# troylee/nnet-asr

Hardware: AMD Instinct MI355X
Metric: training frames/sec (whole node), 440→2048×4→senone MLP, 1/2/4/8 MI355X (higher is better)
Workload: dtype f32; 1 GPU; TNet SGD step, 440x2048x2048x2048x2048x4000 sigmoid MLP + softmax xent; bunch_per_gpu=1024, global_bunch=1024, frames_resident_per_gpu=65536, parallelism=dp1

## Files before the change

### include/tnet_kernels.h

```cpp
#ifndef TNET_KERNELS_H_
#define TNET_KERNELS_H_

#ifdef __cplusplus
extern "C" {
#endif

typedef struct TnetMatrixDim_ {
  int rows;
  int cols;
  int stride;
} TnetMatrixDim;

#define TNET_STATS_SLOTS 512
#define TNET_STATS_WORDS (2 * TNET_STATS_SLOTS)

enum {
  TNET_OK = 0,
  TNET_ERR_ARG = -1,
  TNET_ERR_LAUNCH = -2,
  TNET_ERR_RUNTIME = -3,
  TNET_ERR_UNSUPPORTED = -4
};

const char* tnet_status_str(int status);
// ... 10 lines not shown
int tnetF_add_scaled_row(float alpha, const float* row, float beta, float* dst, TnetMatrixDim d, void* stream);
int tnetF_mul_elem(float* mat, const float* A, int strideA, TnetMatrixDim d, void* stream);
int tnetF_log_elem(float* mat, TnetMatrixDim d, void* stream);

long tnet_col_sum_workspace(TnetMatrixDim d);
int tnetF_add_col_sum(float alpha, const float* mat, float beta, float* vec, TnetMatrixDim d, void* workspace,
                      void* stream);

int tnetF_sigmoid(float* y, const float* x, TnetMatrixDim d, void* stream);
int tnetF_diff_sigmoid(float* eout, const float* e, const float* y, TnetMatrixDim d, void* stream);
int tnetF_softmax(float* y, const float* x, TnetMatrixDim d, void* stream);
int tnetF_check_class(const float* out, const float* des, int* match, TnetMatrixDim d, void* stream);

int tnetF_expand(float* y, const float* x, const int* off, TnetMatrixDim dout, TnetMatrixDim din, void* stream);
int tnetF_rearrange(float* y, const float* x, const int* copy_from, TnetMatrixDim dout, TnetMatrixDim din,
                    void* stream);
int tnet_block_linearity(float* y, TnetMatrixDim dy, const float* x, TnetMatrixDim dx, const float* t,
                         TnetMatrixDim dt, void* stream);
int tnetF_randomize(float* y, const float* x, const int* copy_from, TnetMatrixDim dout, TnetMatrixDim din,
                    void* stream);
int tnet_gather_i32(int* out, const int* in, const int* copy_from, int n, void* stream);
int tnet_gather_bunch(float* y, const float* x, int* labels_out, const int* labels_in, const int* copy_from,
                      TnetMatrixDim dout, TnetMatrixDim din, void* stream);

int tnet_sgemm(char transa, char transb, int m, int n, int k, float alpha, const float* A, int lda,
               const float* B, int ldb, float beta, float* C, int ldc, void* stream);
int tnet_gemm_config(const char* name);
int tnet_gemm_reserve(int cus);

int tnet_affine_fwd(const float* X, TnetMatrixDim dX, const float* W, TnetMatrixDim dW, const float* b,
                    float* Y, TnetMatrixDim dY, int act, void* stream);
int tnet_affine_fwd_sample(const float* X, TnetMatrixDim dX, const float* W, TnetMatrixDim dW, const float* b,
                           float* Y, TnetMatrixDim dY, float* states, int ld_states, unsigned* z1, unsigned* z2,
                           unsigned* z3, unsigned* z4, void* stream);
int tnet_affine_fwd_t(const float* X, TnetMatrixDim dX, const float* W, TnetMatrixDim dW, const float* b,
                      float* Y, TnetMatrixDim dY, int act, void* stream);
int tnet_affine_bwd(const float* E, TnetMatrixDim dE, const float* W, TnetMatrixDim dW, const float* Ybelow,
                    int strideYbelow, float* Eo, TnetMatrixDim dEo, int dsig, void* stream);
int tnet_affine_update(const float* X, TnetMatrixDim dX, const float* E, TnetMatrixDim dE, float* W,
                       TnetMatrixDim dW, float* corrW, int strideCorr, float scale, float mmt, float l2,
                       void* stream);
int tnet_colsum_slabs(int rows);
int tnet_affine_bwd_colsum(const float* E, TnetMatrixDim dE, const float* W, TnetMatrixDim dW,
                           const float* Ybelow, int strideYbelow, float* Eo, TnetMatrixDim dEo, float* colpart,
                           int ldcolpart, void* stream);
int tnet_colsum_slab_sums(const float* E, TnetMatrixDim dE, float* colpart, int ldcolpart, void* stream);
#define TNET_AFFINE_SOFTMAX_MAX_N 256
int tnet_affine_softmax_xent(const float* X, TnetMatrixDim dX, const float* W, TnetMatrixDim dW, const float* b,
                             const int* labels, float* Z, int strideZ, float* Y, int strideY, float* E, int strideE,
                             double* stats, float* colpart, int ldcolpart, void* stream);
int tnet_affine_update_bias(const float* X, TnetMatrixDim dX, const float* E, TnetMatrixDim dE, float* W,
                            TnetMatrixDim dW, float* corrW, int strideCorr, float scale, float mmt, float l2,
                            const float* colpart, int ldcolpart, float* b, float* corr_b, void* stream);
int tnet_affine_update_bwd_pair(const float* X, TnetMatrixDim dX, const float* E, TnetMatrixDim dE, float* W,
                                TnetMatrixDim dW, float* corrW, int strideCorr, float scale, float mmt, float l2,
                                const float* colpart, int ldcolpart, float* b, float* corr_b, const float* E2,
                                TnetMatrixDim dE2, const float* W2, TnetMatrixDim dW2, const float* Ybelow,
                                int strideYbelow, float* Eo, TnetMatrixDim dEo, float* colpart2, int ldcolpart2,
                                void* stream);
int tnet_affine_update_bias_pair(const float* X, TnetMatrixDim dX, const float* E, TnetMatrixDim dE, float* W,
                                 TnetMatrixDim dW, float* corrW, int strideCorr, float scale, float mmt, float l2,
                                 const float* colpart, int ldcolpart, float* b, float* corr_b, const float* X2,
                                 TnetMatrixDim dX2, const float* E2, TnetMatrixDim dE2, float* W2, TnetMatrixDim dW2,
                                 float* corrW2, int strideCorr2, float scale2, float mmt2, float l22,
                                 const float* colpart2, int ldcolpart2, float* b2, float* corr_b2, void* stream);
int tnet_affine_bwd_colsum_slabs(const float* E, TnetMatrixDim dE, const float* W, TnetMatrixDim dW,
                                 const float* Ybelow, int strideYbelow, float* Eo, TnetMatrixDim dEo, float* colpart,
                                 int ldcolpart, float* colpartE, int ldcolpartE, void* stream);
int tnet_affine_bwd_colsum_t(const float* E, TnetMatrixDim dE, const float* Wt, TnetMatrixDim dWt, const float* Ybelow,
                             int strideYbelow, float* Eo, TnetMatrixDim dEo, float* colpart, int ldcolpart,
                             void* stream);
int tnet_affine_bwd_colsum_slabs_t(const float* E, TnetMatrixDim dE, const float* Wt, TnetMatrixDim dWt,
                                   const float* Ybelow, int strideYbelow, float* Eo, TnetMatrixDim dEo, float* colpart,
                                   int ldcolpart, float* colpartE, int ldcolpartE, void* stream);
int tnet_affine_update_bwd_pair_t(const float* X, TnetMatrixDim dX, const float* E, TnetMatrixDim dE, float* W,
                                  TnetMatrixDim dW, float* corrW, int strideCorr, float scale, float mmt, float l2,
                                  const float* colpart, int ldcolpart, float* b, float* corr_b, const float* E2,
                                  TnetMatrixDim dE2, const float* W2t, TnetMatrixDim dW2t, const float* Ybelow,
                                  int strideYbelow, float* Eo, TnetMatrixDim dEo, float* colpart2, int ldcolpart2,
                                  void* stream);
int tnet_weight_shadow(const float* W, TnetMatrixDim dW, float* Wt, int ldwt);
int tnet_weight_shadow_kept(const float* W);
int tnet_transpose(const float* A, TnetMatrixDim dA, float* T, int ldt, void* stream);
int tnet_affine_update_bias_gather(const float* X, TnetMatrixDim dX, const float* E, TnetMatrixDim dE, float* W,
                                   TnetMatrixDim dW, float* corrW, int strideCorr, float scale, float mmt, float l2,
                                   const float* colpart, int ldcolpart, float* b, float* corr_b, const float* X2,
                                   TnetMatrixDim dX2, const float* E2, TnetMatrixDim dE2, float* W2,
                                   TnetMatrixDim dW2, float* corrW2, int strideCorr2, float scale2, float mmt2,
                                   float l22, const float* colpart2, int ldcolpart2, float* b2, float* corr_b2,
                                   float* y, const float* x, int* labels_out, const int* labels_in,
                                   const int* copy_from, TnetMatrixDim dy, TnetMatrixDim dx, void* stream);
int tnet_affine_grad(const float* X, TnetMatrixDim dX, const float* E, TnetMatrixDim dE, float* G,
                     TnetMatrixDim dG, void* stream);
int tnet_affine_grad_bias(const float* X, TnetMatrixDim dX, const float* E, TnetMatrixDim dE, float* G,
                          TnetMatrixDim dG, const float* colpart, int ldcolpart, float* gradB, void* stream);
int tnet_affine_grad_bwd_pair(const float* X, TnetMatrixDim dX, const float* E, TnetMatrixDim dE, float* G,
                              TnetMatrixDim dG, const float* colpart, int ldcolpart, float* gradB, const float* E2,
                              TnetMatrixDim dE2, const float* W2, TnetMatrixDim dW2, const float* Ybelow,
                              int strideYbelow, float* Eo, TnetMatrixDim dEo, float* colpart2, int ldcolpart2,
                              void* stream);
int tnet_affine_grad_bias_gather(const float* X, TnetMatrixDim dX, const float* E, TnetMatrixDim dE, float* G,
                                 TnetMatrixDim dG, const float* colpart, int ldcolpart, float* gradB, const float* X2,
                                 TnetMatrixDim dX2, const float* E2, TnetMatrixDim dE2, float* G2, TnetMatrixDim dG2,
                                 const float* colpart2, int ldcolpart2, float* gradB2, float* y, const float* x,
                                 int* labels_out, const int* labels_in, const int* copy_from, TnetMatrixDim dy,
                                 TnetMatrixDim dx, void* stream);
int tnet_sgd_update(float* p, const float* g, float* corr, long n, float scale, float mmt, float l2,
                    void* stream);
typedef struct TnetSgdSeg_ {
  float* p;
  const float* g;
  float* corr;
  long n;
  float l2;
} TnetSgdSeg;
int tnet_sgd_update_multi(const TnetSgdSeg* segs, int nseg, float scale, float mmt, void* stream);
int tnet_bias_update(const float* E, TnetMatrixDim dE, float* b, float* corr_b, float* grad_out, float scale,
                     float mmt, void* workspace, void* stream);
int tnet_rbm_update(const float* V, TnetMatrixDim dV, const float* H, TnetMatrixDim dH, float* W,
                    TnetMatrixDim dW, float* corrW, int strideCorr, float scale, float mmt, float l2,
                    void* stream);
int tnet_rbm_bias_update(const float* M, TnetMatrixDim d, int neg_from, float* b, float* corr_b, float scale,
                         float mmt, void* workspace, void* stream);
int tnet_rbm_update_stats(const float* V, TnetMatrixDim dV, const float* H, TnetMatrixDim dH, float* W,
                          TnetMatrixDim dW, float* corrW, int strideCorr, float scale, float mmt, float l2, int B,
                          float* vb, float* cvb, float* hb, float* chb, double* mse_stats, void* stream);
int tnet_rbm_update_stats_gather(const float* V, TnetMatrixDim dV, const float* H, TnetMatrixDim dH, float* W,
                                 TnetMatrixDim dW, float* corrW, int strideCorr, float scale, float mmt, float l2,
                                 int B, float* vb, float* cvb, float* hb, float* chb, double* mse_stats, float* y,
                                 const float* x, int* labels_out, const int* labels_in, const int* copy_from,
                                 TnetMatrixDim dy, TnetMatrixDim dx, void* stream);
int tnet_rbm_stats_update(const float* Vs, TnetMatrixDim dV, const float* Hs, TnetMatrixDim dH, int B, float* vb,
                          float* cvb, float* hb, float* chb, float scale, float mmt, double* mse_stats, void* stream);

int tnet_gemv_rowvec_cat(const float* v0, int K0, const float* v1, int K1, float* vout, const float* W, int ldw,
                         const float* b, float* y, int N, int act, void* workspace, void* stream);
int tnet_gemv_rowvec_softmax_xent(const float* v, int K, const float* W, int ldw, const float* b, float* z, float* y,
                                  float* e, int N, const int* label, double* stats, void* workspace, void* stream);
int tnet_gemv_rowvec_partial(const float* v0, int K0, const float* v1, int K1, float* vout, const float* W, int ldw,
                             int N, float* partial, void* stream);
int tnet_rnn_out_partial(const float* hpart, int hslices, const float* hb, float* h, int H, const float* Wo, int ldwo,
                         int N, float* opart, void* stream);
int tnet_rnn_out_stats(const float* opart, int H, int N, const float* bo, float* z, double* smx, void* stream);
int tnet_rnn_out_full(const float* hpart, int hslices, const float* hb, float* h, int H, const float* Wo, int ldwo,
                      int N, const float* bo, float* z, double* smx, void* stream);
int tnet_gemv_rowvec_partial_update(const float* v0, int K0, const float* v1, int K1, float* vout, float* W, int ldw,
                                    int N, float* partial, const float* hist, int ldh, int head, int R, const float* D,
                                    int ldd, int steps, float* b, float* corr_b, float lr, float mmt, float wc,
                                    void* stream);
int tnet_rnn_out_bwd_update(const float* z, const double* smx, int pairs, int N, const int* label, const float* h,
                            int H, float* Wo, int ldwo, float* corrWo, int ldc, float* bo, float* corr_bo, float scale,
                            float mmt, float l2, float* y, float* e, float* e_out, float* d, double* stats,
                            unsigned long long* argkey, int train, void* stream);
int tnet_argmax_correct(const unsigned long long* keys, const int* labels, int T, int N, double* stats,
                        void* stream);
int tnet_rnn_out_full_ahead(const float* hpart, int hslices, const float* hb, float* h, int H, const float* Wo,
                            int ldwo, int N, const float* bo, float* z, double* smx, const float* dpart, const float* D,
                            int ldd, int steps, float lr, float mmt, float wc, const float* cb, float* bnext,
                            float* cbnext, float* W, int ldw, int rows, const float* hist, int ldh, int head, int R,
                            void* stream);
int tnet_rnn_out_bwd_update_ahead(const float* z, const double* smx, int pairs, int N, const int* label,
                                  const float* h, int H, float* Wo, int ldwo, float* corrWo, int ldc, float* bo,
                                  float* corr_bo, float scale, float mmt, float l2, float* e, float* eo, float* d,
                                  double* stats, unsigned long long* argkey, const float* bnext, const float* cbnext,
                                  float* b, float* cb, const float* x_next, int nIn, const float* W, int ldw,
                                  float* partial, float* dpart, float* vout, const float* hist, int ldh, int head,
// ... 78 lines not shown
```

### include/tnet_train.h

```cpp
#ifndef TNET_TRAIN_H_
#define TNET_TRAIN_H_

#include <stddef.h>

#include "tnet_kernels.h"

#ifdef __cplusplus
extern "C" {
#endif

typedef struct TnetNetwork TnetNetwork;
typedef struct TnetObjective TnetObjective;
typedef struct TnetTrainer TnetTrainer;
typedef struct TnetComm TnetComm;
typedef struct TnetRbmTrainer TnetRbmTrainer;
typedef struct TnetRnnTrainer TnetRnnTrainer;

const char* tnet_last_error(void);

int tnet_device_count(int* n);
int tnet_select_gpu(int gpu_id);
int tnet_synchronize(void);
void* tnet_stream(void);
int tnet_malloc(void** p, size_t bytes);
int tnet_free(void* p);
int tnet_memcpy_h2d(void* dst, const void* src, size_t bytes);
int tnet_memcpy_d2h(void* dst, const void* src, size_t bytes);
int tnet_memcpy_d2d(void* dst, const void* src, size_t bytes);
int tnet_memset(void* dst, int value, size_t bytes);
int tnet_set_profile(int on);
int tnet_profile_report(char* buf, int cap);
int tnet_kernel_timing(int on);
int tnet_kernel_timing_filter(const char* filter);
int tnet_kernel_timing_report(char* buf, int cap);
int tnet_timer_start(void);
int tnet_timer_stop(float* ms);

TnetNetwork* tnet_net_read(const char* path);
TnetNetwork* tnet_net_read_text(const char* text);
int tnet_net_write(TnetNetwork* net, const char* path);
int tnet_net_free(TnetNetwork* net);
int tnet_net_num_components(TnetNetwork* net);
int tnet_net_component(TnetNetwork* net, int i, char* tag, int cap, int* n_in, int* n_out);
int tnet_net_get_params(TnetNetwork* net, int i, float* W, float* b);
int tnet_net_set_params(TnetNetwork* net, int i, const float* W, const float* b);
int tnet_net_set_learn_rate(TnetNetwork* net, float lr, const char* factors);
int tnet_net_set_momentum(TnetNetwork* net, float mmt);
int tnet_net_set_weightcost(TnetNetwork* net, float wc);
int tnet_net_set_grad_div_frm(TnetNetwork* net, int div);
int tnet_net_propagate(TnetNetwork* net, const float* dX, int rows, int ldx, float* dY, int ldy);
int tnet_net_backpropagate(TnetNetwork* net, const float* dE, int rows, int lde);
int tnet_net_train_bunch(TnetNetwork* net, TnetObjective* obj, const float* dX, int rows, int ldx,
                         const int* dLabels, int train);
int tnet_net_keep_output(TnetNetwork* net, int keep);
int tnet_net_output(TnetNetwork* net, int i, float* host, int ld);

TnetObjective* tnet_obj_create(int type);
int tnet_obj_free(TnetObjective* obj);
int tnet_obj_evaluate(TnetObjective* obj, const float* dOut, int rows, int cols, int ldo, const float* dDes,
                      int ldd, float* dErr, int lde);
int tnet_obj_evaluate_labels(TnetObjective* obj, const float* dOut, int rows, int cols, int ldo,
                             const int* dLabels, float* dErr, int lde);
int tnet_obj_stats(TnetObjective* obj, double* error, long* frames, double* correct);
int tnet_obj_report(TnetObjective* obj, char* buf, int cap);
int tnet_obj_reset(TnetObjective* obj);

TnetTrainer* tnet_trainer_create(TnetNetwork* net, TnetObjective* obj, int bunchsize, int cachesize, long seed,
                                 int randomize, int crossval);
int tnet_trainer_free(TnetTrainer* t);
int tnet_trainer_add_utterance(TnetTrainer* t, const float* feats, int rows, int cols, int ld, const int* labels);
int tnet_trainer_finish(TnetTrainer* t);
long tnet_trainer_steps(TnetTrainer* t);
int tnet_trainer_replay(TnetTrainer* t, long nsteps);
long tnet_trainer_prefill(TnetTrainer* t, const float* feats, int rows, int cols, int ld, const int* labels);
int tnet_debug_fail_train_bunch(long n);
int tnet_trainer_set_comm(TnetTrainer* t, TnetComm* comm);
long tnet_trainer_empty_steps(TnetTrainer* t);
int tnet_trainer_trace(TnetTrainer* t, int trace);
int tnet_trainer_set_transform(TnetTrainer* t, TnetNetwork* transform, int start_ext, int end_ext);

typedef struct TnetFeatureReader TnetFeatureReader;
TnetFeatureReader* tnet_reader_create(const char* scp, int swap, int start_ext, int end_ext, int target_kind,
                                      int deriv_order, const int* deriv_win, const char* mlf, const char* label_map,
                                      const char* label_dir, const char* label_ext, int threads, int depth);
TnetFeatureReader* tnet_reader_create_norm(const char* scp, int swap, int start_ext, int end_ext, int target_kind,
                                           int deriv_order, const int* deriv_win, const char* mlf,
                                           const char* label_map, const char* label_dir, const char* label_ext,
                                           const char* cmn_dir, const char* cmn_mask, const char* cvn_dir,
                                           const char* cvn_mask, const char* cvg_file, int threads, int depth);
int tnet_reader_free(TnetFeatureReader* r);
long tnet_reader_size(TnetFeatureReader* r);
int tnet_reader_next(TnetFeatureReader* r, const float** feats, int* rows, int* cols, const int** labels,
                     int* n_labels, int* samp_period, int* kind, char* logical, int logical_cap);
int tnet_reader_rewind(TnetFeatureReader* r);
int tnet_htk_read(const char* record, int swap, int start_ext, int end_ext, float* out, long cap, int* rows, int* cols,
                  int* samp_period, int* kind);
int tnet_mask_match(const char* mask, const char* label, char* captured, int cap);
int tnet_mlf_lookup(const char* const* patterns, int n_patterns, const char* const* labels, int n_labels,
                    int* rec_out);
long tnet_trainer_add_reader(TnetTrainer* t, TnetFeatureReader* r, long max_utts);

int tnet_net_rbm_get(TnetNetwork* net, int i, float* W, float* vis_bias, float* hid_bias, int* types);
int tnet_net_rbm_set(TnetNetwork* net, int i, const float* W, const float* vis_bias, const float* hid_bias,
                     int vis_type, int hid_type);
int tnet_net_rbm_update(TnetNetwork* net, int i, const float* pos_vis, const float* pos_hid, const float* neg_vis,
                        const float* neg_hid, int rows, int ld_vis, int ld_hid);
TnetRbmTrainer* tnet_rbm_trainer_create(TnetNetwork* net, int bunchsize, int cachesize, long seed, int randomize,
                                        float learn_rate, float momentum, float weightcost);
int tnet_rbm_trainer_free(TnetRbmTrainer* t);
int tnet_rbm_trainer_add_utterance(TnetRbmTrainer* t, const float* feats, int rows, int cols, int ld);
int tnet_rbm_trainer_finish(TnetRbmTrainer* t);
long tnet_rbm_trainer_steps(TnetRbmTrainer* t);
int tnet_rbm_trainer_stats(TnetRbmTrainer* t, double* mse, long* frames);
int tnet_rbm_trainer_report(TnetRbmTrainer* t, char* buf, int cap);
long tnet_rbm_trainer_prefill(TnetRbmTrainer* t, const float* feats, int rows, int cols, int ld);
int tnet_rbm_trainer_replay(TnetRbmTrainer* t, long nsteps);

int tnet_net_recurrent_get(TnetNetwork* net, int i, float* W, float* b);
int tnet_net_recurrent_set(TnetNetwork* net, int i, const float* W, const float* b);
TnetRnnTrainer* tnet_rnn_trainer_create(TnetNetwork* net, TnetObjective* obj, int bptt, int crossval);
int tnet_rnn_trainer_free(TnetRnnTrainer* t);
int tnet_rnn_trainer_utterance(TnetRnnTrainer* t, const float* feats, int rows, int cols, int ld, const int* labels);
long tnet_rnn_trainer_frames(TnetRnnTrainer* t);

int tnet_net_shared_get(TnetNetwork* net, int i, float* W, float* b, int* n_inst);
int tnet_net_shared_set(TnetNetwork* net, int i, const float* W, const float* b);

int tnet_net_discrete_blocks(TnetNetwork* net, int i, int* n_blocks, int* n_in, int* n_out);
// ... 32 lines not shown
```

### nnet-asr_amd/csrc/host/capi.cpp

```cpp
#include <cstring>
#include <fstream>
#include <memory>
#include <sstream>
#include <string>

#include "tnet_train.h"
#include "curbm.h"
#include "curecurrent.h"
#include "cudiscrete.h"
#include "cushared.h"
#include "cusparse.h"
#include "htkio.h"
#include "trainer.h"

using namespace TNet;

static thread_local std::string g_last_error;

#define TRY_BEGIN try {
#define TRY_END                              \
  }                                          \
  catch (std::exception & e) {               \
    g_last_error = e.what();                 \
    return TNET_ERR_RUNTIME;                 \
// ... 121 lines not shown
  TRY_END
}

int tnet_kernel_timing(int on) {
  TRY_BEGIN CuDevice::Instantiate().KernelTiming(on == 2 ? 2 : on != 0 ? 1 : 0);
  TRY_END
}
int tnet_kernel_timing_filter(const char* filter) {
  TRY_BEGIN CuDevice::Instantiate().KernelTimingFilter(filter ? filter : "");
  TRY_END
}
int tnet_kernel_timing_report(char* buf, int cap) {
  TRY_BEGIN std::string s = CuDevice::Instantiate().KTCollect();
  if ((int)s.size() >= cap) Error("tnet_kernel_timing_report: buffer too small");
  std::strncpy(buf, s.c_str(), (size_t)cap);
  TRY_END
}

static hipEvent_t g_t0 = nullptr, g_t1 = nullptr;
int tnet_timer_start(void) {
  TRY_BEGIN if (!g_t0) {
    TNET_HIP_CALL(hipEventCreate(&g_t0));
    TNET_HIP_CALL(hipEventCreate(&g_t1));
  }
  TNET_HIP_CALL(hipEventRecord(g_t0, CuDevice::Instantiate().Stream()));
  TRY_END
}
int tnet_timer_stop(float* ms) {
  TRY_BEGIN TNET_HIP_CALL(hipEventRecord(g_t1, CuDevice::Instantiate().Stream()));
  TNET_HIP_CALL(hipEventSynchronize(g_t1));
  TNET_HIP_CALL(hipEventElapsedTime(ms, g_t0, g_t1));
  TRY_END
}

TnetNetwork* tnet_net_read(const char* path) {
  try {
    std::unique_ptr<TnetNetwork> h(new TnetNetwork);
    h->net.ReadNetwork(path);
    return h.release();
  }
  TRY_END_PTR
}
TnetNetwork* tnet_net_read_text(const char* text) {
  try {
    std::unique_ptr<TnetNetwork> h(new TnetNetwork);
    std::istringstream is(text);
    h->net.ReadNetwork(is);
    return h.release();
  }
  TRY_END_PTR
}
int tnet_net_write(TnetNetwork* h, const char* path) {
  TRY_BEGIN h->net.WriteNetwork(path);
  TRY_END
}
int tnet_net_free(TnetNetwork* h) {
  TRY_BEGIN delete h;
  TRY_END
}
int tnet_net_num_components(TnetNetwork* h) { return h ? h->net.Layers() : TNET_ERR_ARG; }
int tnet_net_component(TnetNetwork* h, int i, char* tag, int cap, int* n_in, int* n_out) {
  TRY_BEGIN if (i < 0 || i >= h->net.Layers()) Error("component index out of range");
  CuComponent& c = h->net.Layer(i);
  if (tag && cap > 0) {
    std::strncpy(tag, c.GetName(), (size_t)cap - 1);
    tag[cap - 1] = 0;
  }
  if (n_in) *n_in = (int)c.GetNInputs();
  if (n_out) *n_out = (int)c.GetNOutputs();
  TRY_END
}
static CuBiasedLinearity& linear(TnetNetwork* h, int i) {
  if (i < 0 || i >= h->net.Layers()) Error("component index out of range");
  auto* p = dynamic_cast<CuBiasedLinearity*>(&h->net.Layer(i));
  if (!p) Error("component is not <biasedlinearity>");
  return *p;
}
int tnet_net_get_params(TnetNetwork* h, int i, float* W, float* b) {
  TRY_BEGIN CuBiasedLinearity& L = linear(h, i);
  if (W) L.Linearity().CopyToHost(W, L.Linearity().Cols());
  if (b) L.Bias().CopyToHost(b);
  TRY_END
}
int tnet_net_set_params(TnetNetwork* h, int i, const float* W, const float* b) {
  TRY_BEGIN CuBiasedLinearity& L = linear(h, i);
  if (W) {
    CuMatrix<BaseFloat>& M = L.Linearity();
    TNET_HIP_CALL(hipMemcpy2DAsync(M.pCUData(), M.Stride() * 4, W, M.Cols() * 4, M.Cols() * 4, M.Rows(),
                                   hipMemcpyHostToDevice, CuDevice::Instantiate().Stream()));
  }
  if (b) TNET_HIP_CALL(hipMemcpyAsync(L.Bias().pCUData(), b, L.Bias().Dim() * 4, hipMemcpyHostToDevice,
                                      CuDevice::Instantiate().Stream()));
  CuDevice::Instantiate().Synchronize();
  TRY_END
}
int tnet_net_set_learn_rate(TnetNetwork* h, float lr, const char* factors) {
  TRY_BEGIN h->net.SetLearnRate(lr, factors);
  TRY_END
}
int tnet_net_set_momentum(TnetNetwork* h, float mmt) {
  TRY_BEGIN h->net.SetMomentum(mmt);
  TRY_END
}
int tnet_net_set_weightcost(TnetNetwork* h, float wc) {
  TRY_BEGIN h->net.SetWeightcost(wc);
  TRY_END
}
int tnet_net_set_grad_div_frm(TnetNetwork* h, int div) {
  TRY_BEGIN h->net.SetGradDivFrm(div != 0);
  TRY_END
}
int tnet_net_propagate(TnetNetwork* h, const float* dX, int rows, int ldx, float* dY, int ldy) {
  TRY_BEGIN CuMatrix<BaseFloat>::MakeView(h->in_view, const_cast<float*>(dX), rows, h->net.GetNInputs(), ldx);
  h->net.Propagate(h->in_view, h->out);
  if (dY)
    TNET_HIP_CALL(hipMemcpy2DAsync(dY, (size_t)ldy * 4, h->out.pCUData(), h->out.Stride() * 4, h->out.Cols() * 4,
                                   h->out.Rows(), hipMemcpyDeviceToDevice, CuDevice::Instantiate().Stream()));
  TRY_END
}
int tnet_net_backpropagate(TnetNetwork* h, const float* dE, int rows, int lde) {
  TRY_BEGIN CuMatrix<BaseFloat>::MakeView(h->err_view, const_cast<float*>(dE), rows, h->net.GetNOutputs(), lde);
  h->net.Backpropagate(h->err_view);
  TRY_END
}
int tnet_net_train_bunch(TnetNetwork* h, TnetObjective* o, const float* dX, int rows, int ldx, const int* dLabels,
                         int train) {
  TRY_BEGIN CuMatrix<BaseFloat>::MakeView(h->in_view, const_cast<float*>(dX), rows, h->net.GetNInputs(), ldx);
  CuVector<int>::MakeView(h->lab_view, const_cast<int*>(dLabels), rows);
  h->net.TrainBunch(h->in_view, h->lab_view, *o->obj, train != 0, train ? h->comm : nullptr);
  TRY_END
}
int tnet_net_set_comm(TnetNetwork* h, TnetComm* c) {
  TRY_BEGIN h->comm = c ? c->ex.get() : nullptr;
  TRY_END
}
int tnet_net_train_empty(TnetNetwork* h, TnetComm* c, long global_rows) {
  TRY_BEGIN if (!c) Error("tnet_net_train_empty: no communicator");
  c->ex->SetStepRows((size_t)global_rows);
  h->net.TrainEmpty(*c->ex);
  c->ex->SetStepRows(0);
  TRY_END
}
int tnet_net_keep_output(TnetNetwork* h, int keep) {
  TRY_BEGIN h->net.KeepOutput(keep != 0);
  TRY_END
}
int tnet_net_output(TnetNetwork* h, int i, float* host, int ld) {
  TRY_BEGIN if (i < 0 || i >= h->net.Layers()) Error("component index out of range");
  h->net.Layer(i).GetOutput().CopyToHost(host, (size_t)ld);
  TRY_END
}

TnetObjective* tnet_obj_create(int type) {
  try {
    std::unique_ptr<TnetObjective> h(new TnetObjective);
    h->obj.reset(CuObjectiveFunction::Factory(type == 1 ? CuObjectiveFunction::MEAN_SQUARE_ERROR
                                                        : CuObjectiveFunction::CROSS_ENTROPY));
    return h.release();
  }
  TRY_END_PTR
}
int tnet_obj_free(TnetObjective* o) {
  TRY_BEGIN delete o;
  TRY_END
}
int tnet_obj_evaluate(TnetObjective* o, const float* dOut, int rows, int cols, int ldo, const float* dDes, int ldd,
// ... 550 lines not shown
```

### nnet-asr_amd/csrc/host/culayers.cpp

```cpp
#include "culayers.h"

#include "gradexchange.h"

#include <cctype>
#include <cstdlib>

namespace TNet {

#define S ((void*)CuDevice::Instantiate().Stream())

static bool next_token(std::streambuf* sb, char* buf, size_t cap) {
  int c = sb->sgetc();
  while (c != EOF && std::isspace(c)) c = sb->snextc();
  if (c == EOF) return false;
  size_t n = 0;
  while (c != EOF && !std::isspace(c)) {
    if (n + 1 < cap) buf[n++] = (char)c;
    c = sb->snextc();
  }
  buf[n] = 0;
  return true;
}

void ReadMatrixFast(std::istream& in, Matrix<BaseFloat>& m) {
// ... 26 lines not shown
  if (in.fail() || n < 0) Error("Failed to read vector from stream: no size");
  v.Init((size_t)n);
  std::streambuf* sb = in.rdbuf();
  char tok[128];
  for (long long i = 0; i < n; i++) {
    if (!next_token(sb, tok, sizeof tok)) Error("Failed to read vector from stream: truncated");
    char* end = nullptr;
    v[(size_t)i] = std::strtof(tok, &end);
    if (end == tok) Error(std::string("Failed to read vector from stream: bad token ") + tok);
  }
}

void CuBiasedLinearity::PropagateFnc(const CuMatrix<BaseFloat>& X, CuMatrix<BaseFloat>& Y) {
  CuProfileScope p("CuBiasedLinearity::Propagate");
  if (X.Rows() == 1) {
    void* ws = CuDevice::Instantiate().Workspace((size_t)tnet_gemv_workspace((int)GetNInputs(), (int)GetNOutputs()));
    TNET_SAFE_CALL(tnet_gemv_rowvec(X.pCUData(), (int)GetNInputs(), mLinearity.pCUData(), (int)mLinearity.Stride(),
                                    mBias.pCUData(), Y.pCUData(), (int)GetNOutputs(), 0, ws, S));
    return;
  }
  TNET_SAFE_CALL(tnet_affine_fwd(X.pCUData(), X.Dim(), mLinearity.pCUData(), mLinearity.Dim(), mBias.pCUData(),
                                 Y.pCUData(), Y.Dim(), 0, S));
}

void CuBiasedLinearity::BackpropagateFnc(const CuMatrix<BaseFloat>& X, CuMatrix<BaseFloat>& Y) {
  CuProfileScope p("CuBiasedLinearity::Backpropagate");
  if (X.Rows() == 1) {
    TNET_SAFE_CALL(tnet_gemv_rows(mLinearity.pCUData(), (int)mLinearity.Stride(), 0, (int)GetNInputs(),
                                  (int)GetNOutputs(), X.pCUData(), Y.pCUData(), 0.0f, nullptr, S));
    return;
  }
  TNET_SAFE_CALL(tnet_affine_bwd(X.pCUData(), X.Dim(), mLinearity.pCUData(), mLinearity.Dim(), nullptr, 0,
                                 Y.pCUData(), Y.Dim(), 0, S));
}

void CuBiasedLinearity::UpdateConstants(size_t rows, float* scale, float* l2) const {
  BaseFloat N = 1;
  if (mGradDivFrm) N = static_cast<BaseFloat>(rows);
  BaseFloat mmt_gain = static_cast<BaseFloat>(1.0 / (1.0 - mMomentum));
  N *= mmt_gain;
  *scale = -mLearningRate / N;
  *l2 = -mLearningRate * mWeightcost * (mGradDivFrm ? 1.0f : (BaseFloat)rows);
}

void CuBiasedLinearity::UpdateFrom(const CuMatrix<BaseFloat>& X, const CuMatrix<BaseFloat>& E) {
  CuProfileScope p("CuBiasedLinearity::Update");
  float scale, l2;
  UpdateConstants(X.Rows(), &scale, &l2);
  const bool mmt = mMomentum != 0.0f;
  if (X.Rows() == 1) {
    TNET_SAFE_CALL(tnet_affine_update_row(X.pCUData(), (int)GetNInputs(), E.pCUData(), (int)GetNOutputs(),
                                          mLinearity.pCUData(), (int)mLinearity.Stride(),
                                          mmt ? mLinearityCorrection.pCUData() : nullptr,
                                          (int)mLinearityCorrection.Stride(), mBias.pCUData(),
                                          mmt ? mBiasCorrection.pCUData() : nullptr, scale, mMomentum, l2, S));
    mShadowValid = false;
    return;
  }
  TnetMatrixDim dE = E.Dim();
  void* ws = CuDevice::Instantiate().Workspace((size_t)tnet_col_sum_workspace(dE));
  {
    KTScope kt("bias_update:" + std::to_string(GetNOutputs()), 4.0 * dE.rows * dE.cols);
    TNET_SAFE_CALL(tnet_bias_update(E.pCUData(), dE, mBias.pCUData(), mmt ? mBiasCorrection.pCUData() : nullptr,
                                    nullptr, scale, mMomentum, ws, S));
  }
  KTScope kt("gemm_upd:" + std::to_string(GetNInputs()) + "x" + std::to_string(GetNOutputs()),
             2.0 * X.Rows() * GetNInputs() * GetNOutputs());
  TNET_SAFE_CALL(tnet_affine_update(X.pCUData(), X.Dim(), E.pCUData(), dE, mLinearity.pCUData(), mLinearity.Dim(),
                                    mmt ? mLinearityCorrection.pCUData() : nullptr,
                                    (int)mLinearityCorrection.Stride(), scale, mMomentum, l2, S));
  NoteUpdate();
}

void CuBiasedLinearity::UseShadow() {
  if (!mShadowOn || mLinearityT.Rows() != mLinearity.Cols() || mLinearityT.Cols() != mLinearity.Rows()) {
    mLinearityT.Init(mLinearity.Cols(), mLinearity.Rows());
    mShadowValid = false;
  }
  DropShadowKey();
  TNET_SAFE_CALL(tnet_weight_shadow(mLinearity.pCUData(), mLinearity.Dim(), mLinearityT.pCUData(),
                                    (int)mLinearityT.Stride()));
  mShadowKey = mLinearity.pCUData();
  mShadowOn = true;
}

void CuBiasedLinearity::DropShadowKey() {
  if (mShadowKey && mShadowKey != mLinearity.pCUData()) {
    (void)tnet_weight_shadow(mShadowKey, TnetMatrixDim{}, nullptr, 0);
    mShadowValid = false;
  }
  mShadowKey = nullptr;
}

const CuMatrix<BaseFloat>& CuBiasedLinearity::ShadowForBwd() {
  if (!mShadowOn) Error("CuBiasedLinearity::ShadowForBwd: no shadow (UseShadow)");
  if (!mShadowValid) {
    KTScope kt("transpose:" + std::to_string(GetNInputs()) + "x" + std::to_string(GetNOutputs()),
               8.0 * GetNInputs() * GetNOutputs());
    TNET_SAFE_CALL(tnet_transpose(mLinearity.pCUData(), mLinearity.Dim(), mLinearityT.pCUData(),
                                  (int)mLinearityT.Stride(), S));
    mShadowValid = true;
  }
  return mLinearityT;
}

void CuBiasedLinearity::BackpropUpdateRow(const CuMatrix<BaseFloat>& X, const CuMatrix<BaseFloat>& E,
                                          CuMatrix<BaseFloat>& Eout, const float* s, float* d) {
  CuProfileScope p("CuBiasedLinearity::BackpropUpdate");
  if (X.Rows() != 1 || E.Rows() != 1) Error("CuBiasedLinearity::BackpropUpdateRow: one frame only");
  float scale, l2;
  UpdateConstants(1, &scale, &l2);
  const bool mmt = mMomentum != 0.0f;
  Eout.Init(1, GetNInputs());
  TNET_SAFE_CALL(tnet_affine_bwd_update_row(X.pCUData(), (int)GetNInputs(), E.pCUData(), (int)GetNOutputs(),
                                            mLinearity.pCUData(), (int)mLinearity.Stride(),
                                            mmt ? mLinearityCorrection.pCUData() : nullptr,
                                            (int)mLinearityCorrection.Stride(), mBias.pCUData(),
                                            mmt ? mBiasCorrection.pCUData() : nullptr, scale, mMomentum, l2,
                                            Eout.pCUData(), s, d, S));
  mShadowValid = false;
}

void CuBiasedLinearity::UpdateFromColsum(const CuMatrix<BaseFloat>& X, const CuMatrix<BaseFloat>& E,
                                         const CuMatrix<BaseFloat>& colpart) {
  CuProfileScope p("CuBiasedLinearity::Update");
  float scale, l2;
  UpdateConstants(X.Rows(), &scale, &l2);
  const bool mmt = mMomentum != 0.0f;
  KTScope kt("gemm_upd:" + std::to_string(GetNInputs()) + "x" + std::to_string(GetNOutputs()),
             2.0 * X.Rows() * GetNInputs() * GetNOutputs());
  TNET_SAFE_CALL(tnet_affine_update_bias(X.pCUData(), X.Dim(), E.pCUData(), E.Dim(), mLinearity.pCUData(),
                                         mLinearity.Dim(), mmt ? mLinearityCorrection.pCUData() : nullptr,
                                         (int)mLinearityCorrection.Stride(), scale, mMomentum, l2, colpart.pCUData(),
                                         (int)colpart.Stride(), mBias.pCUData(),
                                         mmt ? mBiasCorrection.pCUData() : nullptr, S));
  NoteUpdate();
}

bool CuBiasedLinearity::UpdateFromColsumWithBwd(const CuMatrix<BaseFloat>& X, const CuMatrix<BaseFloat>& E,
                                                const CuMatrix<BaseFloat>& colpart, const CuBiasedLinearity& below,
                                                const CuMatrix<BaseFloat>& E2, const CuMatrix<BaseFloat>& Ybelow,
                                                CuMatrix<BaseFloat>& Eo, CuMatrix<BaseFloat>& colpart2,
                                                bool use_shadow) {
  CuProfileScope p("CuBiasedLinearity::Update+Backpropagate");
  float scale, l2;
  UpdateConstants(X.Rows(), &scale, &l2);
  const bool mmt = mMomentum != 0.0f;
  const std::string su = std::to_string(GetNInputs()) + "x" + std::to_string(GetNOutputs());
  const std::string sb = std::to_string(below.GetNInputs()) + "x" + std::to_string(below.GetNOutputs());
  KTScope kt("gemm_upd+bwd:" + (su == sb ? su : su + "+" + sb),
             2.0 * X.Rows() * GetNInputs() * GetNOutputs() + 2.0 * E2.Rows() * below.GetNInputs() * below.GetNOutputs(),
             2);
  const CuMatrix<BaseFloat>* wt =
      use_shadow && below.HasShadow() ? &const_cast<CuBiasedLinearity&>(below).ShadowForBwd() : nullptr;
  auto pair = wt ? tnet_affine_update_bwd_pair_t : tnet_affine_update_bwd_pair;
  const CuMatrix<BaseFloat>& wb = wt ? *wt : below.LinearityRO();
  const int st = pair(
      X.pCUData(), X.Dim(), E.pCUData(), E.Dim(), mLinearity.pCUData(), mLinearity.Dim(),
      mmt ? mLinearityCorrection.pCUData() : nullptr, (int)mLinearityCorrection.Stride(), scale, mMomentum, l2,
      colpart.pCUData(), (int)colpart.Stride(), mBias.pCUData(), mmt ? mBiasCorrection.pCUData() : nullptr,
      E2.pCUData(), E2.Dim(), wb.pCUData(), wb.Dim(), Ybelow.pCUData(),
      (int)Ybelow.Stride(), Eo.pCUData(), Eo.Dim(), colpart2.pCUData(), (int)colpart2.Stride(), S);
  if (st == TNET_ERR_UNSUPPORTED) {
    kt.Cancel();
    return false;
  }
// ... 268 lines not shown
```

### nnet-asr_amd/csrc/host/culayers.h

```cpp
#pragma once

#include "cucomponent.h"

namespace TNet {

class CuBiasedLinearity : public CuUpdatableComponent {
 public:
  CuBiasedLinearity(size_t nInputs, size_t nOutputs, CuComponent* pPred)
      : CuUpdatableComponent(nInputs, nOutputs, pPred),
        mLinearity(nInputs, nOutputs), mBias(nOutputs),
        mLinearityCorrection(nInputs, nOutputs), mBiasCorrection(nOutputs) {}
  ~CuBiasedLinearity() {
    if (mShadowKey) (void)tnet_weight_shadow(mShadowKey, TnetMatrixDim{}, nullptr, 0);
  }

  ComponentType GetType() const override { return BIASED_LINEARITY; }
  const char* GetName() const override { return "<biasedlinearity>"; }

  void PropagateFnc(const CuMatrix<BaseFloat>& X, CuMatrix<BaseFloat>& Y) override;
  void BackpropagateFnc(const CuMatrix<BaseFloat>& X, CuMatrix<BaseFloat>& Y) override;
  void Update() override;
  void ComputeGradient() override;
  void ComputeGradientColsum(const CuMatrix<BaseFloat>& colpart);
  bool ComputeGradientColsumGather(const CuMatrix<BaseFloat>& colpart, const BunchGather& g,
                                   CuBiasedLinearity* other = nullptr, const CuMatrix<BaseFloat>* colpart2 = nullptr);
  bool ComputeGradientColsumWithBwd(const CuMatrix<BaseFloat>& colpart, const CuBiasedLinearity& below,
                                    const CuMatrix<BaseFloat>& E2, const CuMatrix<BaseFloat>& Ybelow,
                                    CuMatrix<BaseFloat>& Eo, CuMatrix<BaseFloat>& colpart2);
  void ApplyGradient(size_t frames, void* stream = nullptr, const GradExchange* ex = nullptr) override;
  static void ApplyGradients(CuBiasedLinearity* const* ls, int n, size_t frames, const GradExchange* ex);
  std::vector<CuParamBlock> GradientBlocks() override;

  void ReadFromStream(std::istream& rIn) override;
  void WriteToStream(std::ostream& rOut) override;

  CuMatrix<BaseFloat>& Linearity() {
    mShadowValid = false;
    return mLinearity;
  }
  const CuMatrix<BaseFloat>& Linearity() const { return mLinearity; }
  const CuMatrix<BaseFloat>& LinearityRO() const { return mLinearity; }
  void UseShadow();
  const CuMatrix<BaseFloat>& ShadowForBwd();
  bool HasShadow() const { return mShadowOn; }
  CuVector<BaseFloat>& Bias() { return mBias; }
  CuMatrix<BaseFloat>& LinearityCorrection() { return mLinearityCorrection; }
  CuVector<BaseFloat>& BiasCorrection() { return mBiasCorrection; }
  void UpdateConstants(size_t rows, float* scale, float* l2) const;
  void UpdateFrom(const CuMatrix<BaseFloat>& X, const CuMatrix<BaseFloat>& E);
  void BackpropUpdateRow(const CuMatrix<BaseFloat>& X, const CuMatrix<BaseFloat>& E, CuMatrix<BaseFloat>& Eout,
                         const float* s, float* d);
  void UpdateFromColsum(const CuMatrix<BaseFloat>& X, const CuMatrix<BaseFloat>& E, const CuMatrix<BaseFloat>& colpart);
  bool UpdatePairFromColsum(const CuMatrix<BaseFloat>& X, const CuMatrix<BaseFloat>& E,
                            const CuMatrix<BaseFloat>& colpart, CuBiasedLinearity& other, const CuMatrix<BaseFloat>& X2,
                            const CuMatrix<BaseFloat>& E2, const CuMatrix<BaseFloat>& colpart2);
  bool UpdateFromColsumGather(const CuMatrix<BaseFloat>& X, const CuMatrix<BaseFloat>& E,
                              const CuMatrix<BaseFloat>& colpart, CuBiasedLinearity* other,
                              const CuMatrix<BaseFloat>* X2, const CuMatrix<BaseFloat>* E2,
                              const CuMatrix<BaseFloat>* colpart2, const BunchGather& g);
  bool UpdateFromColsumWithBwd(const CuMatrix<BaseFloat>& X, const CuMatrix<BaseFloat>& E,
                               const CuMatrix<BaseFloat>& colpart, const CuBiasedLinearity& below,
                               const CuMatrix<BaseFloat>& E2, const CuMatrix<BaseFloat>& Ybelow,
                               CuMatrix<BaseFloat>& Eo, CuMatrix<BaseFloat>& colpart2, bool use_shadow);

 protected:
  CuMatrix<BaseFloat> mLinearity;
  CuVector<BaseFloat> mBias;
  CuMatrix<BaseFloat> mLinearityCorrection;
  CuVector<BaseFloat> mBiasCorrection;
  CuMatrix<BaseFloat> mGradW;
  CuVector<BaseFloat> mGradB;
  CuMatrix<BaseFloat> mLinearityT;
  bool mShadowOn = false, mShadowValid = false;
  const float* mShadowKey = nullptr;
  void DropShadowKey();
  void NoteUpdate() { mShadowValid = mShadowOn && tnet_weight_shadow_kept(mLinearity.pCUData()) == 1; }
  int ApplySegments(size_t frames, const GradExchange* ex, TnetSgdSeg* seg, float* scale);
};

class CuSigmoid : public CuComponent {
 public:
  CuSigmoid(size_t nInputs, size_t nOutputs, CuComponent* pPred) : CuComponent(nInputs, nOutputs, pPred) {}
  ComponentType GetType() const override { return SIGMOID; }
  const char* GetName() const override { return "<sigmoid>"; }

 protected:
  void PropagateFnc(const CuMatrix<BaseFloat>& X, CuMatrix<BaseFloat>& Y) override;
  void BackpropagateFnc(const CuMatrix<BaseFloat>& X, CuMatrix<BaseFloat>& Y) override;
};

class CuSoftmax : public CuComponent {
 public:
  CuSoftmax(size_t nInputs, size_t nOutputs, CuComponent* pPred) : CuComponent(nInputs, nOutputs, pPred) {}
  ComponentType GetType() const override { return SOFTMAX; }
  const char* GetName() const override { return "<softmax>"; }

 protected:
  void PropagateFnc(const CuMatrix<BaseFloat>& X, CuMatrix<BaseFloat>& Y) override;
  void BackpropagateFnc(const CuMatrix<BaseFloat>& X, CuMatrix<BaseFloat>& Y) override;
};

void ReadMatrixFast(std::istream& in, Matrix<BaseFloat>& m);
void ReadVectorFast(std::istream& in, Vector<BaseFloat>& v);

}
```

### nnet-asr_amd/csrc/host/cunetwork.cpp

```cpp
#include "cunetwork.h"

#include "cufeat.h"
#include "curbm.h"
#include "curecurrent.h"
#include "cudiscrete.h"
#include "cushared.h"
#include "cusparse.h"

#include <algorithm>
#include <cctype>
#include <fstream>
#include <list>

#include "gradexchange.h"

namespace TNet {

#define S ((void*)CuDevice::Instantiate().Stream())

CuNetwork::~CuNetwork() {
  for (auto*& c : mNetComponents) {
    delete c;
    c = nullptr;
  }
// ... 200 lines not shown
    if (c == mpPropagErrorStopper) break;
  }
}

void CuNetwork::DataParallelBackward(GradExchange& exchange, size_t grows, bool empty) {
  std::vector<CuUpdatableComponent*> submitted;
  int n_submitted = 0;
  for (auto it = mNetComponents.rbegin(); it != mNetComponents.rend(); ++it) {
    CuComponent* c = *it;
    const bool stopper = c == mpPropagErrorStopper;
    if (!empty && !stopper) c->Backpropagate();
    if (c->IsUpdatable()) {
      auto* u = static_cast<CuUpdatableComponent*>(c);
      if (u->LearnRate() > 0.0f) {
        if (empty) u->ZeroGradient();
        else u->ComputeGradient();
        exchange.Submit(*u);
        void* as = submitted.empty() ? exchange.ApplyStream(n_submitted) : nullptr;
        if (as) {
          u->ApplyGradient(grows, as, &exchange);
          exchange.GatherParams(*u, n_submitted, as);
        } else {
          submitted.push_back(u);
        }
        n_submitted++;
      }
    }
    if (stopper) break;
  }
  const int first = n_submitted - (int)submitted.size();
  for (size_t i = 0; i < submitted.size(); i++) {
    exchange.WaitFor(first + (int)i);
    submitted[i]->ApplyGradient(grows, nullptr, &exchange);
    exchange.GatherParams(*submitted[i], first + (int)i, nullptr);
  }
  exchange.WaitAll();
}

void CuNetwork::TrainEmpty(GradExchange& exchange) {
  if (!IsFusableMLP()) {
    CheckDataParallel(exchange);
    DataParallelBackward(exchange, exchange.GlobalRows(0), true);
    return;
  }
  const int nl = (int)mNetComponents.size() / 2;
  const size_t grows = exchange.GlobalRows(0);
  std::vector<CuBiasedLinearity*> submitted;
  int n_submitted = 0;
  for (int l = nl - 1; l >= 0; l--) {
    auto* lin = static_cast<CuBiasedLinearity*>(mNetComponents[2 * l]);
    if (lin->LearnRate() > 0.0f) {
      lin->ZeroGradient();
      exchange.Submit(*lin);
      void* as = submitted.empty() ? exchange.ApplyStream(n_submitted) : nullptr;
      if (as) {
        lin->ApplyGradient(grows, as, &exchange);
        exchange.GatherParams(*lin, n_submitted, as);
      } else {
        submitted.push_back(lin);
      }
      n_submitted++;
    }
    if (lin == mpPropagErrorStopper) break;
  }
  const int first = n_submitted - (int)submitted.size();
  for (size_t i = 0; i < submitted.size(); i++) {
    exchange.WaitFor(first + (int)i);
    submitted[i]->ApplyGradient(grows, nullptr, &exchange);
    exchange.GatherParams(*submitted[i], first + (int)i, nullptr);
  }
  exchange.WaitAll();
}

void CuUpdatableComponent::ZeroGradient() {
  for (auto& b : GradientBlocks())
    TNET_HIP_CALL(hipMemsetAsync(b.grad, 0, (size_t)b.n * sizeof(float), CuDevice::Instantiate().Stream()));
}

static long g_fail_train_bunch = 0;
void CuNetwork::DebugFailTrainBunch(long n) { g_fail_train_bunch = n; }

static const bool g_dp_pair = !(getenv("TNET_DP_PAIR") && getenv("TNET_DP_PAIR")[0] == '0');

void CuNetwork::TrainBunch(const CuMatrix<BaseFloat>& X, const CuVector<int>& labels, CuObjectiveFunction& obj,
                           bool train, GradExchange* exchange) {
  if (g_fail_train_bunch > 0 && --g_fail_train_bunch == 0) Error("CuNetwork::TrainBunch: injected fault");
  if (!IsFusableMLP() || obj.GetTypeId() != CuObjectiveFunction::CROSS_ENTROPY) {
    if (!exchange || !train) {
      TrainBunchGeneric(X, labels, obj, train);
      return;
    }
    if (IsFusableMLP()) Error("CuNetwork::TrainBunch: data-parallel training of the sigmoid MLP needs cross-entropy");
    CheckDataParallel(*exchange);
    CuMatrix<BaseFloat> out;
    Propagate(X, out);
    obj.EvaluateLabels(out, labels, mGlobErr);
    mNetComponents.back()->SetErrorInput(mGlobErr);
    DataParallelBackward(*exchange, exchange->GlobalRows(X.Rows()), false);
    return;
  }
  if (X.Cols() != GetNInputs()) Error("CuNetwork::TrainBunch: non-matching input dim");
  if (labels.Dim() != X.Rows()) Error("CuNetwork::TrainBunch: number of labels != rows");
  const size_t rows = X.Rows();
  const int nl = (int)mNetComponents.size() / 2;
  if (mErr.size() != (size_t)nl) {
    mErr.clear();
    mColPart.clear();
    for (int l = 0; l < nl; l++) {
      mErr.emplace_back(new CuMatrix<BaseFloat>());
      mColPart.emplace_back(new CuMatrix<BaseFloat>());
    }
  }
  mNetComponents.front()->SetInput(X);
  static const int use_shadow = getenv("TNET_BWD_SHADOW") ? atoi(getenv("TNET_BWD_SHADOW")) : 2;
  const bool shadows = use_shadow > 0 && train && !exchange;
  if (shadows)
    for (int l = 1; l < (use_shadow == 2 ? nl - 1 : nl); l++)
      static_cast<CuBiasedLinearity*>(mNetComponents[2 * l])->UseShadow();

  CuComponent* smx = mNetComponents.back();
  float* yout = nullptr;
  int ystride = 0;
  if (mKeepOutput) {
    smx->Output().Init(rows, smx->GetNOutputs());
    yout = smx->Output().pCUData();
    ystride = (int)smx->Output().Stride();
  }
  mGlobErr.Init(rows, GetNOutputs());
  auto* top = static_cast<CuBiasedLinearity*>(mNetComponents[2 * (nl - 1)]);
  const bool top_colsum = train && top->LearnRate() > 0.0f;
  bool err_colsum = false;

  const CuMatrix<BaseFloat>* act = &X;
  std::vector<const CuMatrix<BaseFloat>*> acts(nl + 1);
  acts[0] = &X;
  bool fused_top = false;
  for (int l = 0; l < nl; l++) {
    auto* lin = static_cast<CuBiasedLinearity*>(mNetComponents[2 * l]);
    CuComponent* actc = mNetComponents[2 * l + 1];
    const bool last = (l == nl - 1);
    CuMatrix<BaseFloat>& dst = last ? lin->Output() : actc->Output();
    dst.Init(rows, lin->GetNOutputs());
    const std::string shape = std::to_string(lin->GetNInputs()) + "x" + std::to_string(lin->GetNOutputs());
    static const bool fuse_top = !(getenv("TNET_FUSED_TOP") && getenv("TNET_FUSED_TOP")[0] == '0');
    if (last && fuse_top && lin->GetNOutputs() <= TNET_AFFINE_SOFTMAX_MAX_N) {
      float* cp = nullptr;
      int ldcp = 0;
      if (top_colsum) {
        mColPart[l]->Init(tnet_colsum_slabs((int)rows), lin->GetNOutputs());
        cp = mColPart[l]->pCUData();
        ldcp = (int)mColPart[l]->Stride();
      }
      KTScope kt("gemm_fwd+softmax:" + shape, 2.0 * rows * lin->GetNInputs() * lin->GetNOutputs());
      const int st = tnet_affine_softmax_xent(act->pCUData(), act->Dim(), lin->LinearityRO().pCUData(),
                                              lin->LinearityRO().Dim(), lin->Bias().pCUData(), labels.pCUData(),
                                              dst.pCUData(), (int)dst.Stride(), yout, ystride, mGlobErr.pCUData(),
                                              (int)mGlobErr.Stride(), obj.DeviceStats(), cp, ldcp, S);
      if (st != TNET_ERR_UNSUPPORTED) {
        TNET_SAFE_CALL(st);
        fused_top = true;
        err_colsum = top_colsum;
        acts[l + 1] = &dst;
        break;
      }
    }
    KTScope kt("gemm_fwd:" + shape, 2.0 * rows * lin->GetNInputs() * lin->GetNOutputs());
    TNET_SAFE_CALL(tnet_affine_fwd(act->pCUData(), act->Dim(), lin->LinearityRO().pCUData(), lin->LinearityRO().Dim(),
                                   lin->Bias().pCUData(), dst.pCUData(), dst.Dim(), last ? 0 : 1, S));
    act = &dst;
    acts[l + 1] = &dst;
  }
  if (!fused_top) {
    CuMatrix<BaseFloat>& logits = mNetComponents[2 * (nl - 1)]->Output();
    KTScope kts("softmax_xent:" + std::to_string(GetNOutputs()),
                (double)rows * GetNOutputs() * 4.0 * (mKeepOutput ? 3 : 2) + rows * 4.0);
    TNET_SAFE_CALL(tnet_softmax_xent(logits.pCUData(), logits.Dim(), labels.pCUData(), yout, ystride, mGlobErr.pCUData(),
                                     (int)mGlobErr.Stride(), obj.DeviceStats(), S));
  }
  obj.AddFrames(rows);
  if (!train) return;

  const CuMatrix<BaseFloat>* err = &mGlobErr;
  std::vector<CuBiasedLinearity*> submitted;
  const size_t grows = exchange ? exchange->GlobalRows(rows) : rows;
  int n_submitted = 0;
  static const bool slabs_ride = !(getenv("TNET_TOP_SLABS_RIDE") && getenv("TNET_TOP_SLABS_RIDE")[0] == '0');
  bool top_slabs_ride = false;
  auto top_slabs_launch = [&]() {
    CuMatrix<BaseFloat>& cp = *mColPart[nl - 1];
    KTScope kt("colsum:" + std::to_string(GetNOutputs()), 4.0 * rows * GetNOutputs());
    const int st = tnet_colsum_slab_sums(mGlobErr.pCUData(), mGlobErr.Dim(), cp.pCUData(), (int)cp.Stride(), S);
    if (st == TNET_ERR_UNSUPPORTED) return false;
    TNET_SAFE_CALL(st);
    return true;
  };
  if (top_colsum && !fused_top && !err_colsum) {
    mColPart[nl - 1]->Init(tnet_colsum_slabs((int)rows), GetNOutputs());
    const bool top_bwd = nl > 1 && mNetComponents[2 * (nl - 1)] != mpPropagErrorStopper &&
                         static_cast<CuBiasedLinearity*>(mNetComponents[2 * (nl - 2)])->LearnRate() > 0.0f;
    if (slabs_ride && top_bwd) top_slabs_ride = err_colsum = true;
    else err_colsum = top_slabs_launch();
  }
  struct Pending {
    CuBiasedLinearity* lin = nullptr;
    const CuMatrix<BaseFloat>* X = nullptr;
    const CuMatrix<BaseFloat>* E = nullptr;
    int l = -1;
  } pend;
  auto flush = [&]() {
    if (!pend.lin) return;
    pend.lin->UpdateFromColsum(*pend.X, *pend.E, *mColPart[pend.l]);
    pend.lin = nullptr;
  };
  static const bool last_on_apply = getenv("TNET_DP_LAST_APPLY_STREAM") && getenv("TNET_DP_LAST_APPLY_STREAM")[0] == '1';
  auto submit_layer = [&](CuBiasedLinearity* lin, bool last) {
    exchange->Submit(*lin);
    void* as = submitted.empty() && (!last || last_on_apply) ? exchange->ApplyStream(n_submitted) : nullptr;
    if (as) {
      lin->ApplyGradient(grows, as, exchange);
      exchange->GatherParams(*lin, n_submitted, as);
    } else {
      submitted.push_back(lin);
    }
    n_submitted++;
  };
  CuBiasedLinearity* pgrad = nullptr;
  int pgrad_l = -1;
  auto flush_grad = [&]() {
    if (!pgrad) return;
    pgrad->ComputeGradientColsum(*mColPart[pgrad_l]);
    submit_layer(pgrad, false);
    pgrad = nullptr;
  };
  for (int l = nl - 1; l >= 0; l--) {
    auto* lin = static_cast<CuBiasedLinearity*>(mNetComponents[2 * l]);
    const bool stopper = (lin == mpPropagErrorStopper);
    CuMatrix<BaseFloat>* eo = nullptr;
    bool eo_colsum = false;
    if (!stopper && l > 0) {
      eo = mErr[l].get();
      eo->Init(rows, lin->GetNInputs());
      const std::string shape = std::to_string(lin->GetNInputs()) + "x" + std::to_string(lin->GetNOutputs());
      auto* below = static_cast<CuBiasedLinearity*>(mNetComponents[2 * (l - 1)]);
      if (below->LearnRate() > 0.0f) {
        CuMatrix<BaseFloat>& cp = *mColPart[l - 1];
        cp.Init(tnet_colsum_slabs((int)rows), lin->GetNInputs());
        if (pgrad && pgrad->ComputeGradientColsumWithBwd(*mColPart[pgrad_l], *lin, *err, *acts[l], *eo, cp)) {
          submit_layer(pgrad, false);
          pgrad = nullptr;
          eo_colsum = true;
        } else if (pend.lin && pend.lin->UpdateFromColsumWithBwd(*pend.X, *pend.E, *mColPart[pend.l], *lin, *err,
// ... 145 lines not shown
```

### nnet-asr_amd/csrc/kernels/gemm_f32.hip

```cpp
#include <float.h>

#include <cstdlib>
#include <array>
#include <cstring>
#include <initializer_list>
#include <map>
#include <mutex>
#include <unordered_map>
#include <type_traits>

#include "kcommon.h"
#include "rbm_stats.h"
#include "gather.h"

namespace tnetk {

enum { EPI_STORE = 0, EPI_BIAS = 1, EPI_BIAS_SIG = 2, EPI_DSIG = 3, EPI_SGD = 4, EPI_BIAS_NSIG = 5,
       EPI_BIAS_NEG = 6, EPI_RBM = 7,
       EPI_DSIG_CS = 8, EPI_SGD_B = 9,
       EPI_STORE_BG = 10,
       EPI_BIAS_SIG_BIN = 11 };
constexpr int kColsumSlabRows = 32;
constexpr int kMaxSplit = 8;
constexpr int epi_base(int e) {
  return e == EPI_DSIG_CS ? EPI_DSIG : e == EPI_SGD_B ? EPI_SGD : e == EPI_STORE_BG ? EPI_STORE
       : e == EPI_BIAS_SIG_BIN ? EPI_BIAS_SIG : e;
}
constexpr bool epi_bias_slabs(int e) { return e == EPI_SGD_B || e == EPI_STORE_BG; }

struct GemmP {
  int M, N, K;
  const float* A; long lda;
  const float* B; long ldb;
  float* C; long ldc;
  float alpha, beta;
  const float* bias;
  const float* aux; long ldaux;
  float* corr; long ldcorr;
  float scale, mmt, l2;
  float* cpart; long ldcpart;
  const float* bpart; long ldbpart; int bslabs;
  float* bvec; float* bcorr;
  float bscale, bmmt;
  int group;
  int diag_noload;
  int ksplit;
  long kstepA, kstepB, slabC;
  int early_issue;
  int wt;
  unsigned* tile_cnt;
  float* bin; long ldbin;
  unsigned* rz[4];
  float* skws;
  float* Ct; long ldct;
};


template <int TM, int TN, int EPI>
__device__ __forceinline__ void epilogue(const GemmP& p, f32x16 (&acc)[TM][TN], int bm, int bn, int wm0, int wn0,
                                         int li, int lh) {
  const int M = p.M, N = p.N;
#pragma unroll
  for (int a = 0; a < TM; ++a) {
#pragma unroll
    for (int b = 0; b < TN; ++b) {
      const int col = bn + wn0 + b * 32 + li;
      if (col >= N) continue;
      float bias_v = 0.f;
      if (EPI == EPI_BIAS || EPI == EPI_BIAS_SIG || EPI == EPI_BIAS_NSIG || EPI == EPI_BIAS_NEG) bias_v = p.bias[col];
#pragma unroll
      for (int r = 0; r < 16; ++r) {
        const int row = bm + wm0 + a * 32 + (r & 3) + 8 * (r >> 2) + 4 * lh;
        if (row >= M) continue;
        float* cp = p.C + (long)row * p.ldc + col;
        const float v = acc[a][b][r];
        if (EPI == EPI_STORE) {
          *cp = (p.beta == 0.f) ? p.alpha * v : p.alpha * v + p.beta * *cp;
        } else if (EPI == EPI_BIAS) {
          *cp = v + bias_v;
        } else if (EPI == EPI_BIAS_SIG) {
          *cp = sigmoidf_ref(v + bias_v);
        } else if (EPI == EPI_BIAS_NSIG) {
          *cp = -sigmoidf_ref(v + bias_v);
        } else if (EPI == EPI_BIAS_NEG) {
          *cp = -(v + bias_v);
        } else if (EPI == EPI_DSIG) {
          const float y = p.aux[(long)row * p.ldaux + col];
          *cp = y * (1.f - y) * v;
        } else if (EPI == EPI_RBM) {
          float* qp = p.corr + (long)row * p.ldcorr + col;
          const float w = *cp;
          const float c = p.mmt * *qp + p.scale * v + p.l2 * w;
          *qp = c;
          *cp = w + c;
        } else {
          float c = v;
          if (p.corr) {
            float* qp = p.corr + (long)row * p.ldcorr + col;
            c = v + p.mmt * *qp;
            *qp = c;
          }
          float w = *cp;
          w = w + p.scale * c;
          w = w + p.l2 * w;
          *cp = w;
        }
      }
    }
  }
}


constexpr int kBiasPreSlabs = 32;
struct BiasPre {
  float v[kBiasPreSlabs];
  float b, q;
};
template <int BN, bool GRAD>
__device__ __forceinline__ void bias_pre_load(const GemmP& p, int bn, BiasPre& bp) {
  const int col = bn + (int)threadIdx.x;
  if ((int)threadIdx.x >= BN || col >= p.N) return;
#pragma unroll
  for (int k = 0; k < kBiasPreSlabs; ++k) bp.v[k] = k < p.bslabs ? p.bpart[(long)k * p.ldbpart + col] : 0.f;
  if (GRAD) return;
  bp.b = p.bvec[col];
  bp.q = p.bcorr ? p.bcorr[col] : 0.f;
}
template <int BN, bool GRAD>
__device__ __forceinline__ void bias_pre_finish(const GemmP& p, int bn, const BiasPre& bp) {
  const int col = bn + (int)threadIdx.x;
  if ((int)threadIdx.x >= BN || col >= p.N) return;
  double s = 0.0;
#pragma unroll
  for (int k = 0; k < kBiasPreSlabs; ++k) s += (double)bp.v[k];
  for (int k = kBiasPreSlabs; k < p.bslabs; ++k) s += (double)p.bpart[(long)k * p.ldbpart + col];
  float g = (float)s;
  if (GRAD) {
// ... 344 lines not shown
      }
      mfmas(kc % NB);
    }
  }
  if (K % BK) {
    __builtin_amdgcn_s_barrier();
    float* st = smem + (nfull % S) * ST_SZ;
    const int k0 = nfull * BK;
    for (int u = threadIdx.x; u < A_SZ / 4; u += NT) {
      int gr, gc;
      if (A_KC) { const int r = u / CH, j = u % CH; gr = bm + r; gc = k0 + 4 * (j ^ swz<BK>(r)); }
      else { const int k = u / (BM / 4); gr = k0 + k; gc = bm + (u % (BM / 4)) * 4; }
      const int rmax = A_KC ? M : K, cmax = A_KC ? K : M;
      f32x4 x = {0.f, 0.f, 0.f, 0.f};
      if (gr < rmax) {
        const float* q = p.A + (long)gr * p.lda + gc;
#pragma unroll
        for (int e = 0; e < 4; ++e) x[e] = (gc + e < cmax) ? q[e] : 0.f;
      }
      *reinterpret_cast<f32x4*>(st + u * 4) = x;
    }
    for (int u = threadIdx.x; u < B_SZ / 4; u += NT) {
      int gr, gc;
      if (B_KC) { const int r = u / CH, j = u % CH; gr = bn + r; gc = k0 + 4 * (j ^ swz<BK>(r)); }
      else { const int k = u / (BN / 4); gr = k0 + k; gc = bn + (u % (BN / 4)) * 4; }
      const int rmax = B_KC ? N : K, cmax = B_KC ? K : N;
      f32x4 x = {0.f, 0.f, 0.f, 0.f};
      if (gr < rmax) {
        const float* q = p.B + (long)gr * p.ldb + gc;
#pragma unroll
        for (int e = 0; e < 4; ++e) x[e] = (gc + e < cmax) ? q[e] : 0.f;
      }
      *reinterpret_cast<f32x4*>(st + A_SZ + u * 4) = x;
    }
    __syncthreads();
#pragma unroll
    for (int kc = 0; kc < KC; ++kc) {
      read_frags(st, kc, kc % NB);
      mfmas(kc % NB);
    }
  }
  if constexpr (epi_bias_slabs(EPI))
    if (bm == 0) bias_pre_finish<BN, EPI == EPI_STORE_BG>(p, bn, bpre);
  epilogue<TM, TN, epi_base(EPI)>(p, acc, bm, bn, wm0, wn0, li, lh);
  if constexpr (EPI == EPI_BIAS_SIG_BIN) binarize_tile<BM, BN, WM * WN * 64>(p, bm, bn);
}


#ifdef TNET_GEMM_STAMP
__device__ unsigned long long g_tnet_stamps[8192 * 6];
#define TNET_STAMP(i)                                                                   \
  do {                                                                                  \
    const unsigned long long tt_ = __builtin_amdgcn_s_memtime();                        \
    if (threadIdx.x == 0 && blockIdx.x < 8192) g_tnet_stamps[blockIdx.x * 6 + (i)] = tt_; \
  } while (0)
#define TNET_STAMP_RT(i)                                                                \
  do {                                                                                  \
    const unsigned long long tt_ = __builtin_amdgcn_s_memrealtime();                    \
    if (threadIdx.x == 0 && blockIdx.x < 8192) g_tnet_stamps[blockIdx.x * 6 + (i)] = tt_; \
  } while (0)
#else
#define TNET_STAMP(i) do { } while (0)
#define TNET_STAMP_RT(i) do { } while (0)
#endif

template <int V>
__device__ __forceinline__ void lds_vec(const float* p, float (&x)[4]) {
  if constexpr (V == 4) {
    const f32x4 v = *reinterpret_cast<const f32x4*>(p);
    x[0] = v[0]; x[1] = v[1]; x[2] = v[2]; x[3] = v[3];
  } else if constexpr (V == 2) {
    const float2 v = *reinterpret_cast<const float2*>(p);
    x[0] = v.x; x[1] = v.y;
  } else {
    x[0] = *p;
  }
}

constexpr int kEpiStreamK = 64;
template <int BM, int BN, int BK, int S, int EPI_T, bool PX>
constexpr int gemm16_smem_floats() {
  return S * (BM + BN) * BK;
}
template <int BM, int BN, int BK, int WM, int WN, int S, int SP, bool A_KC, bool B_KC, int EPI_T, bool PX>
__device__ __forceinline__ void gemm16_body(const GemmP& p_in, float* __restrict__ smem, const int bid_x) {
  constexpr bool SKM = EPI_T >= kEpiStreamK;
  constexpr int EPI = SKM ? EPI_T - kEpiStreamK : EPI_T;
  GemmP p = p_in;
  if (!SKM && p.ksplit > 1) {
    const long z = blockIdx.y;
    p.A += z * p.kstepA;
    p.B += z * p.kstepB;
    p.C += z * p.slabC;
  }
  constexpr int NT = WM * WN * 64, NW = WM * WN;
  constexpr bool LDR = SP == 2;
  constexpr bool DIR = SP >= 3;
  constexpr int DD = (SP == 3 || SP == 5 || SP == 9) ? 4 : SP == 7 ? 2 : 8;
  static_assert(SP != 1 || S >= 3, "spread DMA needs a 3-slot ring");
  constexpr int WTM = BM / WM, WTN = BN / WN;
  constexpr int TM = WTM / 16, TN = WTN / 16;
  static_assert(WTM % 16 == 0 && WTN % 16 == 0, "16x16 tiles per wave");
  constexpr int VM = A_KC ? 1 : (TM % 4 == 0 ? 4 : TM % 2 == 0 ? 2 : 1);
  constexpr int VN = B_KC ? 1 : (TN % 4 == 0 ? 4 : TN % 2 == 0 ? 2 : 1);
  constexpr int NRA = A_KC ? TM : 4 * TM / VM, NRB = B_KC ? TN : 4 * TN / VN;
  static_assert(BK == 32 || BK == 64, "BK");
  constexpr int CH = BK / 4, KCH = BK / 16;
  constexpr int A_SZ = BM * BK, B_SZ = BN * BK, ST_SZ = A_SZ + B_SZ;
  constexpr int GA = A_SZ / 4 / NT, GB = B_SZ / 4 / NT, G = GA + GB;
  static_assert(A_SZ % (4 * NT) == 0 && B_SZ % (4 * NT) == 0, "tile splits into 1-KiB wave pieces");
  static_assert(3 * G < 64, "vmcnt range");
  TNET_STAMP_RT(4);
  TNET_STAMP(0);

  const int M = p.M, N = p.N, K = p.K;
  const int nbn = (N + BN - 1) / BN, nbm = (M + BM - 1) / BM;
  const int nwg = nbm * nbn;
  const int bid = bid_x, xcd = bid & 7, q8 = nwg >> 3, r8 = nwg & 7;
  const int L = SKM ? bid : (xcd < r8 ? xcd * (q8 + 1) : r8 * (q8 + 1) + (xcd - r8) * q8) + (bid >> 3);
  const int grp = p.group, per_group = grp * nbn;
  const int first_m = (L / per_group) * grp;
  const int gsz = min(nbm - first_m, grp);
  const int bm = (first_m + (L % per_group) % gsz) * BM, bn = ((L % per_group) / gsz) * BN;

  const int lane = threadIdx.x & 63, wid = __builtin_amdgcn_readfirstlane(threadIdx.x >> 6);
  const int wm0 = (wid / WN) * WTM, wn0 = (wid % WN) * WTN;
  const int lg = lane >> 4, li = lane & 15;

  if constexpr (LDR) {
    if (wid == NW) {
      constexpr int GAL = A_SZ / 256, GBL = B_SZ / 256, GL = GAL + GBL;
      static_assert((S - 2) * GL < 64, "loader vmcnt range");
      unsigned offA[GAL], offB[GBL];
#pragma unroll
      for (int g = 0; g < GAL; ++g) {
        const int u = g * 64 + lane;
        if (A_KC) {
          const int r = u / CH, j = u % CH;
          offA[g] = 4u * (unsigned)(min(bm + r, M - 1) * p.lda + 4 * (j ^ swz<BK>(r)));
        } else {
          const int k = u / (BM / 4), c = (u % (BM / 4)) * 4;
          offA[g] = 4u * (unsigned)(k * p.lda + (bm + c < M ? bm + c : 0));
        }
      }
#pragma unroll
      for (int g = 0; g < GBL; ++g) {
        const int u = g * 64 + lane;
        if (B_KC) {
          const int r = u / CH, j = u % CH;
          offB[g] = 4u * (unsigned)(min(bn + r, N - 1) * p.ldb + 4 * (j ^ swz<BK>(r)));
        } else {
          const int k = u / (BN / 4), c = (u % (BN / 4)) * 4;
          offB[g] = 4u * (unsigned)(k * p.ldb + (bn + c < N ? bn + c : 0));
        }
      }
      auto issue_l = [&](int t, int sl) {
        float* st = smem + sl * ST_SZ;
        const char* ab = (const char*)(p.A + (A_KC ? (long)t * BK : (long)t * BK * p.lda));
        const char* bb = (const char*)(p.B + (B_KC ? (long)t * BK : (long)t * BK * p.ldb));
#pragma unroll
        for (int g = 0; g < GAL; ++g) {
          unsigned o = offA[g];
          asm volatile("" : "+v"(o));
          __builtin_amdgcn_global_load_lds((const void*)(ab + o), (void*)(st + g * 256), 16, 0, 0);
        }
#pragma unroll
        for (int g = 0; g < GBL; ++g) {
// ... 329 lines not shown
#pragma unroll
        for (int s2 = 0; s2 < 4; ++s2) av[buf][a][s2] = x[s2];
      } else {
        const int s2 = r % 4, q = r / 4;
        float x[4];
        lds_vec<VM>(As + (16 * c + 4 * lg + s2) * BM + wm0 + 16 * VM * q + VM * li, x);
#pragma unroll
        for (int e = 0; e < VM; ++e) av[buf][VM * q + e][s2] = x[e];
      }
    } else {
      const int rb = r - NRA;
      if (B_KC) {
        const int b = rb, col = wn0 + 16 * b + li;
        const f32x4 x = *reinterpret_cast<const f32x4*>(Bs + col * BK + 4 * ((4 * c + lg) ^ swz<BK>(col)));
#pragma unroll
        for (int s2 = 0; s2 < 4; ++s2) bv[buf][b][s2] = x[s2];
      } else {
        const int s2 = rb % 4, q = rb / 4;
        float x[4];
        lds_vec<VN>(Bs + (16 * c + 4 * lg + s2) * BN + wn0 + 16 * VN * q + VN * li, x);
#pragma unroll
        for (int e = 0; e < VN; ++e) bv[buf][VN * q + e][s2] = x[e];
      }
    }
  };
  auto issue_one = [&](int t, int sl, int g) {
    float* st = smem + sl * ST_SZ;
    if (g < GA) {
      const char* ab = (const char*)(p.A + (A_KC ? (long)t * BK : (long)t * BK * p.lda));
      unsigned o = srcA[g];
      asm volatile("" : "+v"(o));
      __builtin_amdgcn_global_load_lds((const void*)(ab + o), (void*)(st + (g * NW + wid) * 256), 16, 0, 0);
    } else {
      const char* bb = (const char*)(p.B + (B_KC ? (long)t * BK : (long)t * BK * p.ldb));
      unsigned o = srcB[g - GA];
      asm volatile("" : "+v"(o));
      __builtin_amdgcn_global_load_lds((const void*)(bb + o), (void*)(st + A_SZ + ((g - GA) * NW + wid) * 256), 16,
                                       0, 0);
    }
  };

  if constexpr (DIR) {
    constexpr int NR = NRA + NRB;
    constexpr bool ASM = SP >= 5 && (A_KC || VM == 4) && (B_KC || VN == 4) && (NR == 6 || NR == 8 || NR == 12);
    constexpr bool CKC = ASM && (SP == 8 || SP == 9) && (A_KC || B_KC);
    constexpr int NKC = (A_KC ? NRA : 0) + (B_KC ? NRB : 0);
    const int rq = CKC ? lane >> 2 : li, kq = CKC ? lane & 3 : lg;
    const __amdgpu_buffer_rsrc_t rA = tile_rsrc(p.A), rB = tile_rsrc(p.B);
    unsigned oA[NRA], oB[NRB];
#pragma unroll
    for (int r = 0; r < NRA; ++r) {
      if (A_KC) {
        oA[r] = 4u * (unsigned)(min(bm + wm0 + 16 * r + rq, M - 1) * p.lda + 4 * kq);
      } else {
        const int s2 = r % 4, q = r / 4;
        oA[r] = 4u * (unsigned)((4 * lg + s2) * p.lda + max(min(bm + wm0 + 16 * VM * q + VM * li, M - VM), 0));
      }
    }
#pragma unroll
    for (int r = 0; r < NRB; ++r) {
      if (B_KC) {
        oB[r] = 4u * (unsigned)(min(bn + wn0 + 16 * r + rq, N - 1) * p.ldb + 4 * kq);
      } else {
        const int s2 = r % 4, q = r / 4;
        oB[r] = 4u * (unsigned)((4 * lg + s2) * p.ldb + max(min(bn + wn0 + 16 * VN * q + VN * li, N - VN), 0));
      }
    }
    const int cA = A_KC ? 64 : 64 * p.lda, cB = B_KC ? 64 : 64 * p.ldb;
    const int nch = nfull * KCH;
    if constexpr (ASM) {
      const unsigned long long ba = (unsigned long long)(uintptr_t)p.A, bb = (unsigned long long)(uintptr_t)p.B;
      const u32x4 dA = {(unsigned)ba, (unsigned)(ba >> 32), 0x7FFFFFF0u, 0x00020000u};
      const u32x4 dB = {(unsigned)bb, (unsigned)(bb >> 32), 0x7FFFFFF0u, 0x00020000u};
      f32x4 ring[DD][NR];
      auto ld = [&](int c, int r) {
        f32x4 v;
        if (r < NRA)
          asm volatile("buffer_load_dwordx4 %0, %1, %2, %3 offen" : "=v"(v) : "v"(oA[r]), "s"(dA), "s"(c * cA));
        else
          asm volatile("buffer_load_dwordx4 %0, %1, %2, %3 offen" : "=v"(v) : "v"(oB[r - NRA]), "s"(dB), "s"(c * cB));
        return v;
      };
      constexpr int WV = (DD - 2) * NR;
      auto wait_slot = [&](f32x4 (&q)[NR]) {
        if constexpr (NR == 6)
          asm volatile("s_waitcnt vmcnt(%6)" : "+v"(q[0]), "+v"(q[1]), "+v"(q[2]), "+v"(q[3]), "+v"(q[4]), "+v"(q[5])
                       : "n"(WV));
        else if constexpr (NR == 8)
          asm volatile("s_waitcnt vmcnt(%8)"
                       : "+v"(q[0]), "+v"(q[1]), "+v"(q[2]), "+v"(q[3]), "+v"(q[4]), "+v"(q[5]), "+v"(q[6]), "+v"(q[7])
                       : "n"(WV));
        else
          asm volatile("s_waitcnt vmcnt(%12)"
                       : "+v"(q[0]), "+v"(q[1]), "+v"(q[2]), "+v"(q[3]), "+v"(q[4]), "+v"(q[5]), "+v"(q[6]), "+v"(q[7]),
                         "+v"(q[8]), "+v"(q[9]), "+v"(q[10]), "+v"(q[11])
                       : "n"(WV));
      };
      const int pperm = 4 * (4 * li + lg);
      auto perm = [&](f32x4& v) {
        f32x4 o;
#pragma unroll
        for (int e = 0; e < 4; ++e)
          o[e] = __int_as_float(__builtin_amdgcn_ds_bpermute(pperm, __float_as_int(v[e])));
        v = o;
      };
      auto kc_reg = [](int t) { return A_KC ? t : NRA + t; };
      static_assert(!CKC || 4 * TM * TN >= NR + NKC, "a chunk's MFMAs cover its loads and the next one's permutes");
#pragma unroll
      for (int j = 0; j < DD - 1; ++j)
#pragma unroll
        for (int r = 0; r < NR; ++r) ring[j][r] = ld(min(j, nch - 1), r);
      if constexpr (CKC) {
        wait_slot(ring[0]);
#pragma unroll
        for (int t = 0; t < NKC; ++t) perm(ring[0][kc_reg(t)]);
      }
      for (int c0 = 0; c0 < nch; c0 += DD) {
#pragma unroll
        for (int j = 0; j < DD; ++j) {
          const int cn = min(c0 + j + DD - 1, nch - 1);
          if constexpr (!CKC) {
            __builtin_amdgcn_sched_barrier(0);
            wait_slot(ring[j]);
            __builtin_amdgcn_sched_barrier(0);
          }
          int mi = 0;
#pragma unroll
          for (int s2 = 0; s2 < 4; ++s2)
#pragma unroll
            for (int a = 0; a < TM; ++a)
#pragma unroll
              for (int b = 0; b < TN; ++b) {
                const float av_ = A_KC ? ring[j][a][s2] : ring[j][(a / 4) * 4 + s2][a % 4];
                const float bv_ = B_KC ? ring[j][NRA + b][s2] : ring[j][NRA + (b / 4) * 4 + s2][b % 4];
                acc[a][b] = __builtin_amdgcn_mfma_f32_16x16x4f32(av_, bv_, acc[a][b], 0, 0, 0);
                if (mi < NR) {
                  __builtin_amdgcn_sched_barrier(0);
                  ring[(j + DD - 1) % DD][mi] = ld(cn, mi);
                  __builtin_amdgcn_sched_barrier(0);
                }
                if constexpr (CKC) {
                  if (mi == NR - 1) {
                    __builtin_amdgcn_sched_barrier(0);
                    wait_slot(ring[(j + 1) % DD]);
                    __builtin_amdgcn_sched_barrier(0);
                  } else if (mi >= NR && mi < NR + NKC) {
                    __builtin_amdgcn_sched_barrier(0);
                    perm(ring[(j + 1) % DD][kc_reg(mi - NR)]);
                    __builtin_amdgcn_sched_barrier(0);
                  }
                }
                ++mi;
              }
        }
      }
      asm volatile("s_waitcnt vmcnt(0)" ::: "memory");
    } else {
    float fa[DD][TM][4], fb[DD][TN][4];
    auto gld = [&](__amdgpu_buffer_rsrc_t rs, unsigned off, int soff, float (&x)[4], auto vtag) {
      constexpr int V = decltype(vtag)::value;
      if constexpr (V == 4) {
        const f32x4 v = __builtin_bit_cast(f32x4, __builtin_amdgcn_raw_buffer_load_b128(rs, (int)off, soff, 0));
        x[0] = v[0]; x[1] = v[1]; x[2] = v[2]; x[3] = v[3];
      } else if constexpr (V == 2) {
        const auto v = __builtin_amdgcn_raw_buffer_load_b64(rs, (int)off, soff, 0);
        x[0] = __uint_as_float(v[0]); x[1] = __uint_as_float(v[1]);
      } else {
        x[0] = __uint_as_float(__builtin_amdgcn_raw_buffer_load_b32(rs, (int)off, soff, 0));
      }
    };
    auto load_one = [&](int c, float (&ra)[TM][4], float (&rb)[TN][4], int r) {
      if (r < NRA) {
        if (A_KC) {
          gld(rA, oA[r], c * cA, ra[r], std::integral_constant<int, 4>{});
        } else {
          const int s2 = r % 4, q = r / 4;
          float x[4];
          gld(rA, oA[r], c * cA, x, std::integral_constant<int, VM>{});
#pragma unroll
          for (int e = 0; e < VM; ++e) ra[VM * q + e][s2] = x[e];
        }
      } else {
        const int rb_ = r - NRA;
        if (B_KC) {
          gld(rB, oB[rb_], c * cB, rb[rb_], std::integral_constant<int, 4>{});
        } else {
          const int s2 = rb_ % 4, q = rb_ / 4;
          float x[4];
          gld(rB, oB[rb_], c * cB, x, std::integral_constant<int, VN>{});
#pragma unroll
          for (int e = 0; e < VN; ++e) rb[VN * q + e][s2] = x[e];
        }
      }
    };
#pragma unroll
    for (int j = 0; j < DD - 1; ++j)
#pragma unroll
      for (int r = 0; r < NR; ++r) load_one(min(j, nch - 1), fa[j], fb[j], r);
    for (int c0 = 0; c0 < nch; c0 += DD) {
#pragma unroll
      for (int j = 0; j < DD; ++j) {
        const int cn = min(c0 + j + DD - 1, nch - 1);
        int mi = 0;
#pragma unroll
        for (int s2 = 0; s2 < 4; ++s2)
#pragma unroll
          for (int a = 0; a < TM; ++a)
#pragma unroll
            for (int b = 0; b < TN; ++b) {
              acc[a][b] = __builtin_amdgcn_mfma_f32_16x16x4f32(fa[j][a][s2], fb[j][b][s2], acc[a][b], 0, 0, 0);
              if (mi < NR) {
                __builtin_amdgcn_sched_barrier(0);
                load_one(cn, fa[(j + DD - 1) % DD], fb[(j + DD - 1) % DD], mi);
                __builtin_amdgcn_sched_barrier(0);
              }
              ++mi;
            }
      }
    }
    }
  } else {
  int sl = 0;
  for (int t = 0; t < nfull; ++t) {
    const float* st = smem + sl * ST_SZ;
    const int sl1 = sl + 1 == S ? 0 : sl + 1;
    const int slp = sl == 0 ? S - 1 : sl - 1;
    const int tsp = min(t + S - 1, tlast), tns = min(t + S, tlast);
#pragma unroll
    for (int c = 0; c < KCH; ++c) {
      const int buf = c & 1;
      const bool seam = c + 1 == KCH;
      const float* rst = seam ? smem + sl1 * ST_SZ : st;
      const int rc = seam ? 0 : c + 1;
      if (seam) {
        __builtin_amdgcn_sched_barrier(0);
        __builtin_amdgcn_s_waitcnt(0xC07F);
// ... 60 lines not shown
    const int k0 = nfull * BK, Kt = K - k0;
#pragma unroll
    for (int g = 0; g < GA; ++g) {
      const int u = (g * NW + wid) * 64 + lane;
      long off;
      if (A_KC) {
        const int r = u / CH, j = u % CH, kc = k0 + 4 * (j ^ swz<BK>(r));
        off = (long)min(bm + r, M - 1) * p.lda + (kc < K ? kc : K - 4);
      } else {
        const int k = u / (BM / 4), c = (u % (BM / 4)) * 4;
        off = (long)min(k0 + k, K - 1) * p.lda + (bm + c < M ? bm + c : 0);
      }
      __builtin_amdgcn_global_load_lds((const void*)(p.A + off), (void*)(st + (g * NW + wid) * 256), 16, 0, 0);
    }
#pragma unroll
    for (int g = 0; g < GB; ++g) {
      const int u = (g * NW + wid) * 64 + lane;
      long off;
      if (B_KC) {
        const int r = u / CH, j = u % CH, kc = k0 + 4 * (j ^ swz<BK>(r));
        off = (long)min(bn + r, N - 1) * p.ldb + (kc < K ? kc : K - 4);
      } else {
        const int k = u / (BN / 4), c = (u % (BN / 4)) * 4;
        off = (long)min(k0 + k, K - 1) * p.ldb + (bn + c < N ? bn + c : 0);
      }
      __builtin_amdgcn_global_load_lds((const void*)(p.B + off), (void*)(st + A_SZ + (g * NW + wid) * 256), 16, 0,
                                       0);
    }
    wait_vmcnt<0>();
    barrier();
#pragma unroll
    for (int c = 0; c < KCH; ++c) {
      if (16 * c >= Kt) break;
      read_frags(st, c, 0);
#pragma unroll
      for (int s2 = 0; s2 < 4; ++s2) {
        const bool ok = 16 * c + 4 * lg + s2 < Kt;
#pragma unroll
        for (int a = 0; a < TM; ++a) av[0][a][s2] = ok ? av[0][a][s2] : 0.f;
#pragma unroll
        for (int b = 0; b < TN; ++b) bv[0][b][s2] = ok ? bv[0][b][s2] : 0.f;
      }
      mfmas(0);
    }
  } else if (K % BK) {
    __builtin_amdgcn_s_waitcnt(0xC07F);
    __builtin_amdgcn_s_barrier();
    float* st = smem + (nfull % S) * ST_SZ;
    const int k0 = nfull * BK;
    for (int u = threadIdx.x; u < A_SZ / 4; u += NT) {
      int gr, gc;
      if (A_KC) { const int r = u / CH, j = u % CH; gr = bm + r; gc = k0 + 4 * (j ^ swz<BK>(r)); }
      else { const int k = u / (BM / 4); gr = k0 + k; gc = bm + (u % (BM / 4)) * 4; }
      const int rmax = A_KC ? M : K, cmax = A_KC ? K : M;
      f32x4 x = {0.f, 0.f, 0.f, 0.f};
      if (gr < rmax) {
        const float* q = p.A + (long)gr * p.lda + gc;
#pragma unroll
        for (int e = 0; e < 4; ++e) x[e] = (gc + e < cmax) ? q[e] : 0.f;
      }
      *reinterpret_cast<f32x4*>(st + u * 4) = x;
    }
    for (int u = threadIdx.x; u < B_SZ / 4; u += NT) {
      int gr, gc;
      if (B_KC) { const int r = u / CH, j = u % CH; gr = bn + r; gc = k0 + 4 * (j ^ swz<BK>(r)); }
      else { const int k = u / (BN / 4); gr = k0 + k; gc = bn + (u % (BN / 4)) * 4; }
      const int rmax = B_KC ? N : K, cmax = B_KC ? K : N;
      f32x4 x = {0.f, 0.f, 0.f, 0.f};
      if (gr < rmax) {
        const float* q = p.B + (long)gr * p.ldb + gc;
#pragma unroll
        for (int e = 0; e < 4; ++e) x[e] = (gc + e < cmax) ? q[e] : 0.f;
      }
      *reinterpret_cast<f32x4*>(st + A_SZ + u * 4) = x;
    }
    __syncthreads();
#pragma unroll
    for (int c = 0; c < KCH; ++c) {
      read_frags(st, c, 0);
      mfmas(0);
    }
  }

  if constexpr (SKM) {
    if (p.ksplit > 1) {
      constexpr int SLICE = BM * BN;
      const __amdgpu_buffer_rsrc_t rw = tile_rsrc(p.skws + (long)bid_x * SLICE);
      __attribute__((address_space(1))) unsigned* cnt =
          (__attribute__((address_space(1))) unsigned*)(p.tile_cnt + bid_x);
      asm volatile("s_waitcnt vmcnt(0)" ::: "memory");
      __syncthreads();
      if (threadIdx.x == 0) {
        const unsigned ticket = __hip_atomic_fetch_add(cnt, 1u, __ATOMIC_RELAXED, __HIP_MEMORY_SCOPE_AGENT);
        smem[0] = (ticket & 0xFFFFu) == 0 ? 0.f : 1.f;
      }
      __syncthreads();
      if (smem[0] == 0.f) {
#pragma unroll
        for (int a = 0; a < TM; ++a)
#pragma unroll
          for (int b = 0; b < TN; ++b) st_wt(rw, ((long)(a * TN + b) * NT + threadIdx.x) * 4, acc[a][b]);
        asm volatile("s_waitcnt vmcnt(0)" ::: "memory");
        __syncthreads();
        if (threadIdx.x == 0) __hip_atomic_fetch_add(cnt, 0x10000u, __ATOMIC_RELAXED, __HIP_MEMORY_SCOPE_AGENT);
        return;
      }
      if (threadIdx.x == 0) {
        while ((__hip_atomic_load(cnt, __ATOMIC_RELAXED, __HIP_MEMORY_SCOPE_AGENT) >> 16) == 0u)
          __builtin_amdgcn_s_sleep(2);
        __hip_atomic_store(cnt, 0u, __ATOMIC_RELAXED, __HIP_MEMORY_SCOPE_AGENT);
      }
      __syncthreads();
      f32x4 t[TM][TN];
#pragma unroll
      for (int a = 0; a < TM; ++a)
#pragma unroll
        for (int b = 0; b < TN; ++b) t[a][b] = ld_sc1(rw, ((long)(a * TN + b) * NT + threadIdx.x) * 4);
#pragma unroll
      for (int a = 0; a < TM; ++a)
#pragma unroll
        for (int b = 0; b < TN; ++b) acc[a][b] = acc[a][b] + t[a][b];
    }
  }
  if constexpr (epi_bias_slabs(EPI) && !PXB)
    if (bm == 0) bias_pre_finish<BN, EPI == EPI_STORE_BG>(p, bn, bpre);
  if constexpr (PXB) {
    static_assert(S * ST_SZ >= kBiasPreSlabs * 8 && WM * WN * 64 == kBiasPreSlabs * 8, "PX bias layout");
    float* bsm = smem;
    const int u = threadIdx.x;
    __builtin_amdgcn_s_waitcnt(0xC07F);
    __syncthreads();
    bsm[u] = (u >> 3) < p.bslabs ? pxb_v : 0.f;
    __syncthreads();
    if (u < pxb_cpw && (bm / BM) * pxb_cpw + u < BN) {
      double sum = 0.0;
#pragma unroll
      for (int k = 0; k < kBiasPreSlabs; ++k) sum += (double)bsm[k * 8 + u];
      float g = (float)sum;
      if constexpr (EPI == EPI_STORE_BG) {
        p.bvec[pxb_col] = g;
      } else {
        if (p.bcorr) {
          g = g + p.bmmt * pxb_q;
          p.bcorr[pxb_col] = g;
        }
        p.bvec[pxb_col] = pxb_b + p.bscale * g;
      }
    }
  }

  if constexpr (!EARLY) prefetch_tiles();
  const __amdgpu_buffer_rsrc_t rs_c = tile_rsrc(p.C + (long)bm * p.ldc + bn);
  const __amdgpu_buffer_rsrc_t rs_q = tile_rsrc(p.corr ? p.corr + (long)bm * p.ldcorr + bn : p.C);
  constexpr bool CS = EPI == EPI_DSIG_CS;
  static_assert(!CS || (A_KC && WTM == kColsumSlabRows), "column sums: k-contiguous A, 32-row wave tiles");
  if constexpr (TRE) {
    __builtin_amdgcn_s_waitcnt(0xC07F);
    __builtin_amdgcn_s_barrier();
    float* wl = smem + wid * WTM * LDT;
#pragma unroll
    for (int a = 0; a < TM; ++a)
#pragma unroll
      for (int b = 0; b < TN; ++b)
#pragma unroll
        for (int r = 0; r < 4; ++r) wl[(16 * a + 4 * lg + r) * LDT + 16 * b + li] = acc[a][b][r];
    float cs4[4] = {0.f, 0.f, 0.f, 0.f};
// ... 161 lines not shown
#pragma unroll
      for (int aq = 0; aq < TM / VM; ++aq)
#pragma unroll
        for (int r = 0; r < 4; ++r) {
          const int rl0 = erow(VM * aq, r) - bm;
#pragma unroll
          for (int j = 0; j < NJ; ++j)
#pragma unroll
            for (int e = 0; e < NE; ++e) {
              const int cl = ecol(j) + e - bn;
              if constexpr (VM == 4) {
                *reinterpret_cast<f32x4*>(ts + cl * LDP + rl0) =
                    f32x4{acc[4 * aq][NE * j + e][r], acc[4 * aq + 1][NE * j + e][r], acc[4 * aq + 2][NE * j + e][r],
                          acc[4 * aq + 3][NE * j + e][r]};
              } else {
#pragma unroll
                for (int m = 0; m < VM; ++m) ts[cl * LDP + rl0 + m] = acc[VM * aq + m][NE * j + e][r];
              }
            }
        }
      __syncthreads();
      const __amdgpu_buffer_rsrc_t rs_t = tile_rsrc(p.Ct + (long)bn * p.ldct + bm);
      for (int u = threadIdx.x; u < BN * Q; u += NT) {
        const int cl = u / Q, q4 = u % Q, col = bn + cl, row0 = bm + 4 * q4;
        if (col >= N || row0 >= M) continue;
        const f32x4 v = *reinterpret_cast<const f32x4*>(ts + cl * LDP + 4 * q4);
        if (row0 + 3 < M) {
          st_wt(rs_t, (long)cl * p.ldct + 4 * q4, v);
        } else {
#pragma unroll
          for (int m = 0; m < 4; ++m)
            if (row0 + m < M) p.Ct[(long)col * p.ldct + row0 + m] = v[m];
        }
      }
    }
  }
  }
  if constexpr (EPI == EPI_BIAS_SIG_BIN) binarize_tile<BM, BN, NT>(p, bm, bn);
  TNET_STAMP(3);
  TNET_STAMP_RT(5);
}

template <int BM, int BN, int BK, int WM, int WN, int S, bool A_KC, bool B_KC, int EPI, int SPK = 0>
__global__ __launch_bounds__(WM * WN * 64)
__attribute__((amdgpu_waves_per_eu((WM * WN + 3) / 4, (WM * WN + 3) / 4)))
void gemm16_sk_kernel(const GemmP p, const int G) {
  __shared__ __attribute__((aligned(16))) float smem[gemm16_smem_floats<BM, BN, BK, S, EPI, true>()];
  const int T = ((p.M + BM - 1) / BM) * ((p.N + BN - 1) / BN), KT = p.K / BK;
  const long I = (long)T * KT;
  const int b = blockIdx.x, xcd = b & 7, q8 = G >> 3, r8 = G & 7;
  const int v = (xcd < r8 ? xcd * (q8 + 1) : r8 * (q8 + 1) + (xcd - r8) * q8) + (b >> 3);
  const long s = (long)v * I / G, e = (long)(v + 1) * I / G;
  for (long k0 = s; k0 < e;) {
    const int t = (int)(k0 / KT);
    const long tb = (long)t * KT, te = tb + KT, k1 = e < te ? e : te;
    if (k0 != s) __syncthreads();
    const int w0 = (int)(((tb + 1) * G - 1) / I), w1 = (int)((te * G - 1) / I);
    GemmP q = p;
    q.ksplit = w1 - w0 + 1;
    const long kk = (k0 - tb) * BK;
    q.A = p.A + (A_KC ? kk : kk * p.lda);
    q.B = p.B + (B_KC ? kk : kk * p.ldb);
    q.K = (int)((k1 - k0) * BK);
    gemm16_body<BM, BN, BK, WM, WN, S, SPK, A_KC, B_KC, kEpiStreamK + EPI, true>(q, smem, t);
    k0 = k1;
  }
}

template <int BM, int BN, bool A_KC, bool B_KC, int EPI, bool PX>
__global__ __launch_bounds__(256) __attribute__((amdgpu_waves_per_eu(1, 1)))
void gemm16_split2_kernel(const GemmP p) {
  __shared__ __attribute__((aligned(16))) float smem[gemm16_smem_floats<BM, BN, 64, 2, EPI, PX>()];
  const int nwg = gridDim.x, b = blockIdx.x, xcd = b & 7, q8 = nwg >> 3, r8 = nwg & 7;
  const int v = (xcd < r8 ? xcd * (q8 + 1) : r8 * (q8 + 1) + (xcd - r8) * q8) + (b >> 3);
  GemmP q = p;
  const long kk = (long)(v & 1) * (p.K / 2);
  q.A = p.A + (A_KC ? kk : kk * p.lda);
  q.B = p.B + (B_KC ? kk : kk * p.ldb);
  q.K = p.K / 2;
  q.ksplit = 2;
  gemm16_body<BM, BN, 64, 2, 2, 2, 0, A_KC, B_KC, kEpiStreamK + EPI, PX>(q, smem, v >> 1);
}

template <int BM, int BN, int BK, int WM, int WN, int S, int SP, bool A_KC, bool B_KC, int EPI_T, bool PX = false>
__global__ __launch_bounds__((WM * WN + (SP == 2)) * 64)
__attribute__((amdgpu_waves_per_eu((WM * WN + (SP == 2) + 3) / 4, (WM * WN + (SP == 2) + 3) / 4)))
void gemm16_kernel(const GemmP p_in) {
  __shared__ __attribute__((aligned(16))) float smem[gemm16_smem_floats<BM, BN, BK, S, EPI_T, PX>()];
  gemm16_body<BM, BN, BK, WM, WN, S, SP, A_KC, B_KC, EPI_T, PX>(p_in, smem, blockIdx.x);
}

template <int BMA, int BNA, bool AKA, bool BKA, int EPIA, bool PXA, int BMB, int BNB, bool AKB, bool BKB, int EPIB,
          bool PXB, int SPA = 0, int SPB = 0, int KTA = 64, int STA = 2>
__global__ __launch_bounds__(256) __attribute__((amdgpu_waves_per_eu(1, 1)))
void gemm16_pair_kernel(const GemmP pa, const GemmP pb, const int na) {
  constexpr int SA = gemm16_smem_floats<BMA, BNA, KTA, STA, EPIA, PXA>(), SB = gemm16_smem_floats<BMB, BNB, 64, 2, EPIB, PXB>();
  __shared__ __attribute__((aligned(16))) float smem[SA > SB ? SA : SB];
  if ((int)blockIdx.x < na) gemm16_body<BMA, BNA, KTA, 2, 2, STA, SPA, AKA, BKA, EPIA, PXA>(pa, smem, blockIdx.x);
  else gemm16_body<BMB, BNB, 64, 2, 2, 2, SPB, AKB, BKB, EPIB, PXB>(pb, smem, (int)blockIdx.x - na);
}

template <int BM, int BN, int BK, int WM, int WN, int S>
__global__ __launch_bounds__(WM * WN * 64) __attribute__((amdgpu_waves_per_eu(1, 1)))
void gemm16_upd_pair_kernel(const GemmP pa, const GemmP pb, const int na) {
  __shared__ __attribute__((aligned(16))) float smem[gemm16_smem_floats<BM, BN, BK, S, EPI_SGD_B, false>()];
  if ((int)blockIdx.x < na) gemm16_body<BM, BN, BK, WM, WN, S, 0, false, false, EPI_SGD_B, false>(pa, smem, blockIdx.x);
  else gemm16_body<BM, BN, BK, WM, WN, S, 0, false, false, EPI_SGD_B, false>(pb, smem, (int)blockIdx.x - na);
}

template <int BM, int BN, int BK, int WM, int WN, int S, int EPI = EPI_SGD_B>
__global__ __launch_bounds__(WM * WN * 64) __attribute__((amdgpu_waves_per_eu(1, 1)))
void gemm16_upd_gather_kernel(const GemmP pa, const GemmP pb, const int na, const int nb, const BunchGatherP g) {
  __shared__ __attribute__((aligned(16))) float smem[gemm16_smem_floats<BM, BN, BK, S, EPI, false>()];
  const int b = blockIdx.x;
  if (b < na) gemm16_body<BM, BN, BK, WM, WN, S, 0, false, false, EPI, false>(pa, smem, b);
  else if (b < na + nb) gemm16_body<BM, BN, BK, WM, WN, S, 0, false, false, EPI, false>(pb, smem, b - na);
  else bunch_gather_block(g, b - na - nb, (int)gridDim.x - na - nb);
}

template <bool BD>
__global__ __launch_bounds__(256) __attribute__((amdgpu_waves_per_eu(1, 1)))
void gemm16_upd_mixed_gather_kernel(const GemmP pa, const GemmP pb, const int na, const int nb, const BunchGatherP g) {
  constexpr int SA = gemm16_smem_floats<128, 128, 64, 2, EPI_SGD_B, true>();
  constexpr int SB = BD ? gemm16_smem_floats<64, 64, 64, 2, EPI_SGD_B, false>()
                        : gemm16_smem_floats<64, 64, 32, 4, EPI_SGD_B, false>();
  __shared__ __attribute__((aligned(16))) float smem[SA > SB ? SA : SB];
  const int b = blockIdx.x;
  if (b < na) {
    gemm16_body<128, 128, 64, 2, 2, 2, 5, false, false, EPI_SGD_B, true>(pa, smem, b);
  } else if (b < na + nb) {
    if constexpr (BD) gemm16_body<64, 64, 64, 2, 2, 2, 5, false, false, EPI_SGD_B, false>(pb, smem, b - na);
    else gemm16_body<64, 64, 32, 4, 1, 4, 0, false, false, EPI_SGD_B, false>(pb, smem, b - na);
  } else {
    bunch_gather_block(g, b - na - nb, (int)gridDim.x - na - nb);
  }
}

template <bool PX, int SP = 0, bool BKC = true>
__global__ __launch_bounds__(256) __attribute__((amdgpu_waves_per_eu(1, 1)))
void gemm16_bwd_slabs_kernel(const GemmP p, const int na, const float* __restrict__ Et, const TnetMatrixDim dEt,
                             float* __restrict__ cpt, const long ldcpt, const int slabs, const int ncb) {
  __shared__ __attribute__((aligned(16))) float smem[gemm16_smem_floats<64, 128, 64, 2, EPI_DSIG_CS, PX>()];
  const int b = blockIdx.x;
  if (b < na) {
    gemm16_body<64, 128, 64, 2, 2, 2, SP, true, BKC, EPI_DSIG_CS, PX>(p, smem, b);
  } else {
    const int c = b - na;
    colsum_partial_block<true>(Et, dEt, cpt, slabs, 0x7fffffff, ldcpt, c % ncb, c / ncb, smem);
  }
}

__global__ __launch_bounds__(256) __attribute__((amdgpu_waves_per_eu(1, 1)))
void gemm16_rbm_update_stats_kernel(const GemmP p, const int na, const float* __restrict__ Vs, TnetMatrixDim dV,
                                    const float* __restrict__ Hs, TnetMatrixDim dH, int B, int nvb,
                                    float* __restrict__ vb, float* __restrict__ cvb, float* __restrict__ hb,
                                    float* __restrict__ chb, float scale, float mmt, double* __restrict__ stats,
                                    int nhb, const BunchGatherP g, const int ng) {
  constexpr int SG = gemm16_smem_floats<64, 64, 32, 4, EPI_RBM, false>();
  __shared__ __attribute__((aligned(16))) float smem[SG > RS_SMEM_FLOATS ? SG : RS_SMEM_FLOATS];
  const int b = blockIdx.x;
  if (b < na) gemm16_body<64, 64, 32, 4, 1, 4, 0, false, false, EPI_RBM, false>(p, smem, b);
  else if (b < na + ng) bunch_gather_block(g, b - na, ng);
  else rbm_stats_block(b - na - ng, smem, Vs, dV, Hs, dH, B, nvb, vb, cvb, hb, chb, scale, mmt, stats, nhb);
}

constexpr bool epi_splittable(int e) { return e != EPI_DSIG_CS && e != EPI_BIAS_SIG_BIN; }

template <int EPI_FULL>
__global__ __launch_bounds__(256) void splitk_reduce_kernel(const GemmP p, const float* __restrict__ P, long slab,
                                                            int splits, int ldp, unsigned main_blocks) {
  if constexpr (epi_bias_slabs(EPI_FULL)) {
    if (blockIdx.x >= main_blocks) {
// ... 487 lines not shown
  splitk_reduce_kernel<EPI><<<main_blocks + bias_blocks, 256, 0, st>>>(pc, ws, slab, ks, ldp, main_blocks);
  TNET_LAUNCH_CHECK();
  return TNET_OK;
}

static int launch_colsum_bwd(const GemmP& p_in, hipStream_t st) {
  if (p_in.M <= 0 || p_in.N <= 0) return TNET_OK;
  int cfg = forced_cfg();
  const bool autocfg = cfg < 0;
  GemmP p = p_in;
  p.group = g_group > 0 ? g_group : 8;
  if (cfg != CFG_m64x128k64s2 && cfg != CFG_m64x64k32s4 && cfg != CFG_m64x64k64s2)
    cfg = (long)cdiv(p.M, 64) * cdiv(p.N, 128) >= 200 ? CFG_m64x128k64s2 : CFG_m64x64k32s4;
  if (cfg == CFG_m64x128k64s2 && launch_sk<64, 128, true, true, EPI_DSIG_CS>(p, st)) {
    TNET_LAUNCH_CHECK();
    return TNET_OK;
  }
  bool ok = false;
  if (cfg == CFG_m64x128k64s2 && autocfg && g_kc >= 2)
    ok = launch_cfg<1, 64, 128, 64, 2, 2, 2, 8, true, true, EPI_DSIG_CS>(p, st);
  else if (cfg == CFG_m64x128k64s2) ok = launch_cfg<1, 64, 128, 64, 2, 2, 2, 0, true, true, EPI_DSIG_CS>(p, st);
  else if (cfg == CFG_m64x64k64s2) ok = launch_cfg<1, 64, 64, 64, 2, 2, 2, 0, true, true, EPI_DSIG_CS>(p, st);
  else ok = launch_cfg<1, 64, 64, 32, 2, 2, 4, 0, true, true, EPI_DSIG_CS>(p, st);
  if (!ok) return TNET_ERR_UNSUPPORTED;
  TNET_LAUNCH_CHECK();
  return TNET_OK;
}

static int launch_colsum_bwd_t(const GemmP& p_in, hipStream_t st) {
  if (p_in.M <= 0 || p_in.N <= 0) return TNET_OK;
  if (g_reserve > 0 || forced_cfg() >= 0) return TNET_ERR_UNSUPPORTED;
  GemmP p = p_in;
  p.group = g_group > 0 ? g_group : 8;
  bool ok;
  if ((long)cdiv(p.M, 64) * cdiv(p.N, 128) >= 200)
    ok = g_direct > 0 ? launch_cfg<1, 64, 128, 64, 2, 2, 2, 6, true, false, EPI_DSIG_CS>(p, st)
                      : launch_cfg<1, 64, 128, 64, 2, 2, 2, 0, true, false, EPI_DSIG_CS>(p, st);
  else
    ok = launch_cfg<1, 64, 64, 32, 2, 2, 4, 0, true, false, EPI_DSIG_CS>(p, st);
  if (!ok) return TNET_ERR_UNSUPPORTED;
  TNET_LAUNCH_CHECK();
  return TNET_OK;
}

struct GemmPlan {
  int cfg, ks;
};
template <bool A_KC>
static GemmPlan plan_gemm(const GemmP& p, bool splittable) {
  int cfg = forced_cfg();
  if (cfg < 0) {
    const long t128 = (long)cdiv(p.M, 128) * cdiv(p.N, 128), t64x128 = (long)cdiv(p.M, 64) * cdiv(p.N, 128);
    const long t128x256 = (long)cdiv(p.M, 128) * cdiv(p.N, 256);
    const long t64 = (long)cdiv(p.M, 64) * cdiv(p.N, 64), t32x64 = (long)cdiv(p.M, 32) * cdiv(p.N, 64);
    if (!A_KC && t128x256 >= 240) cfg = CFG_m128x256k32s3;
    else if (t128 >= 240) cfg = CFG_m128x128k64s2;
    else if (A_KC && t64x128 >= 200) cfg = CFG_m64x128k64s2;
    else if (t64 >= 200) cfg = CFG_m64x64k32s4w41;
    else if (A_KC && t32x64 >= 128) cfg = CFG_m32x64k64s2;
    else cfg = CFG_m64x64k32s4w41;
  }
  int ks = 1;
  if (splittable) {
    int tbm, tbn, kind;
    cfg_shape(cfg, &tbm, &tbn, &kind);
    const long tiles = (long)cdiv(p.M, tbm) * cdiv(p.N, tbn);
    if (g_split > 0) {
      ks = g_split < kMaxSplit ? g_split : kMaxSplit;
    } else if (tiles < 100 && p.K >= 1024) {
      while (ks < kMaxSplit && tiles * ks * 2 <= 288) ks *= 2;
      const long t32 = (long)cdiv(p.M, 32) * cdiv(p.N, 64);
      if (cfg == CFG_m64x64k32s4w41 && ks >= 4 && t32 * (ks / 2) <= 288) {
        cfg = CFG_m32x64k64s2;
        kind = 1;
        ks /= 2;
      }
    }
    while (ks > 1 && (p.K % (4 * ks) != 0 || p.K / ks < 64)) ks /= 2;
    if (ks > 1 && kind != 1) cfg = CFG_m64x64k32s4w41;
  }
  return GemmPlan{cfg, ks};
}

template <bool A_KC, bool B_KC, int EPI>
static int launch_gemm(const GemmP& p_in, hipStream_t st) {
  if constexpr (EPI == EPI_DSIG_CS) {
    if constexpr (B_KC) return launch_colsum_bwd(p_in, st);
    else return launch_colsum_bwd_t(p_in, st);
  } else {
  if (p_in.M <= 0 || p_in.N <= 0) return TNET_OK;
  static const int noload = getenv("TNET_GEMM_DIAG") ? atoi(getenv("TNET_GEMM_DIAG")) : 0;
  GemmP p = p_in;
  p.diag_noload = noload;
  p.group = g_group > 0 ? g_group : 8;
  if (launch_split2<A_KC, B_KC, EPI>(p, st)) {
    TNET_LAUNCH_CHECK();
    return TNET_OK;
  }
  const GemmPlan pl = plan_gemm<A_KC>(p, epi_splittable(EPI));
  const int cfg = pl.cfg;
  if (pl.ks > 1) return launch_splitk<A_KC, B_KC, EPI>(p, cfg, pl.ks, st);
  bool sk_done = false;
  if (cfg == CFG_m64x128k64s2) sk_done = launch_sk<64, 128, A_KC, B_KC, EPI>(p, st);
  else if (cfg == CFG_m128x128k64s2) sk_done = launch_sk<128, 128, A_KC, B_KC, EPI>(p, st);
  if (sk_done) {
    TNET_LAUNCH_CHECK();
    return TNET_OK;
  }
  int rcfg = cfg;
  if (g_direct > 0 && forced_cfg() < 0 && !B_KC) {
    if (cfg == CFG_m64x128k64s2)
      rcfg = (g_direct == 3 || p.K <= 512) ? CFG_m64x128a4 : CFG_m64x128a8;
    else if (cfg == CFG_m128x128k64s2) rcfg = CFG_m128x128a4;
    else if (cfg == CFG_m128x256k32s3 && g_direct == 4) rcfg = CFG_m128x256a2;
  }
  if (g_kc >= 2 && forced_cfg() < 0 && A_KC && B_KC && cfg == CFG_m64x128k64s2) rcfg = CFG_m64x128c8;
  if constexpr (!A_KC && !B_KC && (EPI == EPI_SGD_B || EPI == EPI_SGD))
    if (forced_cfg() < 0 && cfg == CFG_m64x64k32s4w41 && upd64_direct(p)) rcfg = CFG_m64x64a4;
  bool ok = false;
  switch (rcfg) {
#define X(name, KIND, BM, BN, BK, WM, WN, S, IL) \
  case CFG_##name: ok = launch_cfg<KIND, BM, BN, BK, WM, WN, S, IL, A_KC, B_KC, EPI>(p, st); break;
    TNET_GEMM_CFGS(X)
#undef X
    default: return TNET_ERR_ARG;
  }
  if (!ok) launch_cfg<0, 64, 64, 32, 2, 2, 4, 0, A_KC, B_KC, EPI>(p, st);
  TNET_LAUNCH_CHECK();
  return TNET_OK;
  }
}

template <int EPIA, bool PXA, int SPA>
static void pair_go(const GemmP& pu, const GemmP& pb, int na, int nb, bool kc, int bt, hipStream_t st) {
  if (bt == 1)
    gemm16_pair_kernel<128, 128, false, false, EPIA, PXA, 64, 128, true, false, EPI_DSIG_CS, true, SPA, 6>
        <<<na + nb, 256, 0, st>>>(pu, pb, na);
  else if (bt == 2)
    gemm16_pair_kernel<128, 128, false, false, EPIA, PXA, 64, 128, true, false, EPI_DSIG_CS, true, SPA, 0>
        <<<na + nb, 256, 0, st>>>(pu, pb, na);
  else if (kc)
    gemm16_pair_kernel<128, 128, false, false, EPIA, PXA, 64, 128, true, true, EPI_DSIG_CS, true, SPA, 8>
        <<<na + nb, 256, 0, st>>>(pu, pb, na);
  else
    gemm16_pair_kernel<128, 128, false, false, EPIA, PXA, 64, 128, true, true, EPI_DSIG_CS, true, SPA>
        <<<na + nb, 256, 0, st>>>(pu, pb, na);
}

static int launch_pair_wide_bwd_t(GemmP pu, GemmP pb, hipStream_t st) {
  static const bool on = !(getenv("TNET_PAIR_WIDE") && getenv("TNET_PAIR_WIDE")[0] == '0');
  if (!on || g_direct != 4 || g_reserve > 0) return TNET_ERR_UNSUPPORTED;
  if ((long)cdiv(pb.M, 64) * cdiv(pb.N, 128) < 200) return TNET_ERR_UNSUPPORTED;
  auto a16p = [](const void* v) { return ((uintptr_t)v & 15) == 0; };
  const bool dir_a = pu.K / 32 >= 1 && pu.M % 4 == 0 && pu.N % 4 == 0 && !(pu.lda & 3) && !(pu.ldb & 3) &&
                     a16p(pu.A) && a16p(pu.B) && 4 * ((long)pu.K * pu.lda) < (1L << 31) &&
                     4 * ((long)pu.K * pu.ldb) < (1L << 31) && 4 * (32L * pu.lda + pu.M) < (1L << 32) &&
                     4 * (32L * pu.ldb + pu.N) < (1L << 32);
  const bool dir_b = pb.K / 64 >= 1 && (pb.K / 64) % 2 == 0 && pb.N % 4 == 0 && !(pb.lda & 3) && !(pb.ldb & 3) &&
                     a16p(pb.A) && a16p(pb.B) && 4 * ((long)pb.M * pb.lda) < (1L << 31) &&
                     4 * ((long)pb.K * pb.ldb) < (1L << 31) && 4 * (64L * pb.ldb + pb.N) < (1L << 32);
  if (!dir_a || !dir_b || !px_exact<64, 128, EPI_DSIG_CS>(pb)) return TNET_ERR_UNSUPPORTED;
  pu.group = pb.group = g_group > 0 ? g_group : 8;
  pu.early_issue = pb.early_issue = g_early;
  pu.wt = pb.wt = g_wt;
  const int na = cdiv(pu.M, 128) * cdiv(pu.N, 256), nb = cdiv(pb.M, 64) * cdiv(pb.N, 128);
  gemm16_pair_kernel<128, 256, false, false, EPI_SGD_B, false, 64, 128, true, false, EPI_DSIG_CS, true, 7, 6, 32, 3>
      <<<na + nb, 256, 0, st>>>(pu, pb, na);
  TNET_LAUNCH_CHECK();
  return TNET_OK;
}

template <int EPIA>
static int launch_pair_a_bwd(GemmP pu, GemmP pb, hipStream_t st, bool bwd_t = false) {
  if (EPIA == EPI_STORE_BG && g_reserve > 0) return TNET_ERR_UNSUPPORTED;
  if (forced_cfg() >= 0 || !g_pair) return TNET_ERR_UNSUPPORTED;
  if (pu.M <= 0 || pu.N <= 0 || pb.M <= 0 || pb.N <= 0) return TNET_ERR_UNSUPPORTED;
  const GemmPlan pl = plan_gemm<false>(pu, true);
  if (EPIA == EPI_SGD_B && bwd_t && pl.cfg == CFG_m128x256k32s3 && pl.ks == 1)
    return launch_pair_wide_bwd_t(pu, pb, st);
  if (pl.cfg != CFG_m128x128k64s2 || pl.ks != 1) return TNET_ERR_UNSUPPORTED;
  if ((long)cdiv(pb.M, 64) * cdiv(pb.N, 128) < 200) return TNET_ERR_UNSUPPORTED;
  pu.group = pb.group = g_group > 0 ? g_group : 8;
  pu.early_issue = pb.early_issue = g_early;
  pu.wt = pb.wt = g_wt;
  const long extA_u = 64L * pu.lda + pu.M, extB_u = 64L * pu.ldb + pu.N;
  const long extA_b = (long)pb.M * pb.lda, extB_b = bwd_t ? 64L * pb.ldb + pb.N : (long)pb.N * pb.ldb;
  if (4 * extA_u >= (1L << 32) || 4 * extB_u >= (1L << 32) || 4 * extA_b >= (1L << 32) || 4 * extB_b >= (1L << 32))
    return TNET_ERR_UNSUPPORTED;
  if (!px_exact<64, 128, EPI_DSIG_CS>(pb)) return TNET_ERR_UNSUPPORTED;
  const int na = cdiv(pu.M, 128) * cdiv(pu.N, 128), nb = cdiv(pb.M, 64) * cdiv(pb.N, 128);
  auto a16p = [](const void* v) { return ((uintptr_t)v & 15) == 0; };
  const bool dir = g_direct > 0 && pu.K / 64 >= 1 && !(pu.lda & 3) && !(pu.ldb & 3) && a16p(pu.A) && a16p(pu.B) &&
                   pu.M % 4 == 0 && pu.N % 4 == 0 &&
                   4 * ((long)pu.K * pu.lda) < (1L << 31) && 4 * ((long)pu.K * pu.ldb) < (1L << 31);
  const bool px = px_exact<128, 128, EPIA>(pu);
  const bool kc = !bwd_t && g_kc >= 2 && kc_direct(pb);
  int bt = 0;
  if (bwd_t) {
// ... 216 lines not shown
  for (const ByteSpan& x : xs)
    for (const ByteSpan& y : ys)
      if (spans_overlap(x, y)) return true;
  return false;
}
static bool gather_independent(float* y, const float* x, int* labels_out, const int* labels_in, const int* copy_from,
                               TnetMatrixDim dy, TnetMatrixDim dx, std::initializer_list<ByteSpan> upd_reads,
                               std::initializer_list<ByteSpan> upd_writes) {
  const ByteSpan gw[] = {span_of(y, dy.rows, dy.stride, 4), span_of(labels_out, dy.rows, 1, 4)};
  const ByteSpan gr[] = {span_of(x, dx.rows, dx.stride, 4), span_of(labels_in, dx.rows, 1, 4),
                         span_of(copy_from, dy.rows, 1, 4)};
  for (const ByteSpan& w : gw) {
    if (any_overlap({w}, upd_reads) || any_overlap({w}, upd_writes)) return false;
    for (const ByteSpan& r : gr)
      if (spans_overlap(w, r)) return false;
  }
  for (const ByteSpan& r : gr)
    if (any_overlap({r}, upd_writes)) return false;
  return true;
}

extern "C" int tnet_rbm_update_stats(const float* V, TnetMatrixDim dV, const float* H, TnetMatrixDim dH, float* W,
                                     TnetMatrixDim dW, float* corrW, int strideCorr, float scale, float mmt, float l2,
                                     int B, float* vb, float* cvb, float* hb, float* chb, double* mse_stats,
                                     void* stream) {
  return rbm_update_stats_run(V, dV, H, dH, W, dW, corrW, strideCorr, scale, mmt, l2, B, vb, cvb, hb, chb, mse_stats,
                              BunchGatherP{}, 0, stream);
}

extern "C" int tnet_rbm_update_stats_gather(const float* V, TnetMatrixDim dV, const float* H, TnetMatrixDim dH,
                                            float* W, TnetMatrixDim dW, float* corrW, int strideCorr, float scale,
                                            float mmt, float l2, int B, float* vb, float* cvb, float* hb, float* chb,
                                            double* mse_stats, float* y, const float* x, int* labels_out,
                                            const int* labels_in, const int* copy_from, TnetMatrixDim dy,
                                            TnetMatrixDim dx, void* stream) {
  if (!y || !x || !labels_out || !labels_in || !copy_from || dy.cols != dx.cols || dy.rows < 0 || dy.stride < dy.cols ||
      dx.stride < dx.cols)
    return TNET_ERR_ARG;
  const int c4 = (dy.cols + 3) & ~3;
  if (((uintptr_t)y & 15) || ((uintptr_t)x & 15) || (dy.stride & 3) || (dx.stride & 3) || c4 > dy.stride ||
      c4 > dx.stride)
    return TNET_ERR_UNSUPPORTED;
  if (!gather_independent(y, x, labels_out, labels_in, copy_from, dy, dx,
                          {span_of(V, dV.rows, dV.stride, 4), span_of(H, dH.rows, dH.stride, 4)},
                          {span_of(W, dW.rows, dW.stride, 4), span_of(corrW, dW.rows, strideCorr, 4),
                           span_of(vb, dV.cols, 1, 4), span_of(cvb, dV.cols, 1, 4), span_of(hb, dH.cols, 1, 4),
                           span_of(chb, dH.cols, 1, 4), span_of(mse_stats, TNET_STATS_WORDS, 1, 8)}))
    return TNET_ERR_ARG;
  return rbm_update_stats_run(V, dV, H, dH, W, dW, corrW, strideCorr, scale, mmt, l2, B, vb, cvb, hb, chb, mse_stats,
                              BunchGatherP{y, x, labels_out, labels_in, copy_from, dy.rows, c4, dy.stride, dx.stride},
                              16, stream);
}

static int rbm_update_stats_run(const float* V, TnetMatrixDim dV, const float* H, TnetMatrixDim dH, float* W,
                                TnetMatrixDim dW, float* corrW, int strideCorr, float scale, float mmt, float l2, int B,
                                float* vb, float* cvb, float* hb, float* chb, double* mse_stats, const BunchGatherP& g,
                                int ng, void* stream) {
  if (dV.rows != dH.rows || dW.rows != dV.cols || dW.cols != dH.cols || !corrW || (strideCorr & 3))
    return TNET_ERR_ARG;
  if (B < 0 || dV.rows != 2 * B || dV.cols <= 0 || dH.cols <= 0 || dV.stride < dV.cols || dH.stride < dH.cols || !vb ||
      !cvb || !hb || !chb)
    return TNET_ERR_ARG;
  if (!B || 2 * B > CS_ROWS * RS_MAX_SLABS || forced_cfg() >= 0 || !g_pair) return TNET_ERR_UNSUPPORTED;
  GemmP p{};
  p.M = dV.cols; p.N = dH.cols; p.K = dV.rows;
  p.A = V; p.lda = dV.stride; p.B = H; p.ldb = dH.stride; p.C = W; p.ldc = dW.stride;
  p.corr = corrW; p.ldcorr = strideCorr;
  p.scale = scale; p.mmt = mmt; p.l2 = l2;
  int st = check_common(p);
  if (st) return st;
  const GemmPlan pl = plan_gemm<false>(p, epi_splittable(EPI_RBM));
  if (pl.cfg != CFG_m64x64k32s4w41 || pl.ks != 1) return TNET_ERR_UNSUPPORTED;
  if (4 * (32L * p.lda + p.M) >= (1L << 32) || 4 * (32L * p.ldb + p.N) >= (1L << 32)) return TNET_ERR_UNSUPPORTED;
  p.group = g_group > 0 ? g_group : 8;
  p.early_issue = g_early;
  p.wt = g_wt;
  const int na = cdiv(p.M, 64) * cdiv(p.N, 64);
  const int nvb = cdiv(dV.cols, RS_COLS), nhb = cdiv(dH.cols, RS_COLS), nmb = mse_stats ? cdiv(B, RS_MROWS) : 0;
  if (ng && cu_count() - g_reserve - na < ng) return TNET_ERR_UNSUPPORTED;
  gemm16_rbm_update_stats_kernel<<<na + ng + nvb + nhb + nmb, 256, 0, (hipStream_t)stream>>>(
      p, na, V, dV, H, dH, B, nvb, vb, cvb, hb, chb, scale, mmt, mse_stats, nhb, g, ng);
  TNET_LAUNCH_CHECK();
  return TNET_OK;
}

extern "C" int tnet_affine_bwd(const float* E, TnetMatrixDim dE, const float* W, TnetMatrixDim dW,
                               const float* Ybelow, int strideYbelow, float* Eo, TnetMatrixDim dEo, int dsig,
                               void* stream) {
  if (dE.cols != dW.cols || dEo.rows != dE.rows || dEo.cols != dW.rows) return TNET_ERR_ARG;
  GemmP p{};
  p.M = dE.rows; p.N = dW.rows; p.K = dE.cols;
  p.A = E; p.lda = dE.stride; p.B = W; p.ldb = dW.stride; p.C = Eo; p.ldc = dEo.stride;
  p.alpha = 1.f; p.beta = 0.f;
  p.aux = Ybelow; p.ldaux = strideYbelow;
  int st = check_common(p);
  if (st) return st;
  if (dsig) {
    if (!Ybelow || !aligned16(Ybelow) || (strideYbelow & 3)) return TNET_ERR_ARG;
    return launch_gemm<true, true, EPI_DSIG>(p, (hipStream_t)stream);
  }
  return launch_gemm<true, true, EPI_STORE>(p, (hipStream_t)stream);
}

extern "C" int tnet_affine_update(const float* X, TnetMatrixDim dX, const float* E, TnetMatrixDim dE, float* W,
                                  TnetMatrixDim dW, float* corrW, int strideCorr, float scale, float mmt,
                                  float l2, void* stream) {
  if (dX.rows != dE.rows || dW.rows != dX.cols || dW.cols != dE.cols) return TNET_ERR_ARG;
  GemmP p{};
  p.M = dX.cols; p.N = dE.cols; p.K = dX.rows;
  p.A = X; p.lda = dX.stride; p.B = E; p.ldb = dE.stride; p.C = W; p.ldc = dW.stride;
  p.corr = (mmt != 0.f || corrW) ? corrW : nullptr; p.ldcorr = strideCorr;
  if (mmt != 0.f && !corrW) return TNET_ERR_ARG;
  if (p.corr && (p.ldcorr & 3)) return TNET_ERR_ARG;
  p.scale = scale; p.mmt = mmt; p.l2 = l2;
  int st = check_common(p);
  if (st) return st;
  shadow_attach(p);
  return shadow_done(p, launch_gemm<false, false, EPI_SGD>(p, (hipStream_t)stream));
}

extern "C" int tnet_colsum_slabs(int rows) { return rows > 0 ? (rows + kColsumSlabRows - 1) / kColsumSlabRows : 0; }

extern "C" int tnet_affine_bwd_colsum(const float* E, TnetMatrixDim dE, const float* W, TnetMatrixDim dW,
                                      const float* Ybelow, int strideYbelow, float* Eo, TnetMatrixDim dEo,
                                      float* colpart, int ldcolpart, void* stream) {
  if (dE.cols != dW.cols || dEo.rows != dE.rows || dEo.cols != dW.rows || !Ybelow || !colpart ||
      ldcolpart < dEo.cols || !aligned16(Ybelow) || (strideYbelow & 3))
    return TNET_ERR_ARG;
  GemmP p{};
  p.M = dE.rows; p.N = dW.rows; p.K = dE.cols;
  p.A = E; p.lda = dE.stride; p.B = W; p.ldb = dW.stride; p.C = Eo; p.ldc = dEo.stride;
  p.alpha = 1.f; p.beta = 0.f;
  p.aux = Ybelow; p.ldaux = strideYbelow;
  p.cpart = colpart; p.ldcpart = ldcolpart;
  int st = check_common(p);
  if (st) return st;
  return launch_gemm<true, true, EPI_DSIG_CS>(p, (hipStream_t)stream);
}

static int bwd_colsum_slabs(const float* E, TnetMatrixDim dE, const float* W, TnetMatrixDim dW, const float* Ybelow,
                            int strideYbelow, float* Eo, TnetMatrixDim dEo, float* colpart, int ldcolpart,
                            float* colpartE, int ldcolpartE, void* stream, bool bt) {
  const int w_k = bt ? dW.rows : dW.cols, w_n = bt ? dW.cols : dW.rows;
  if (dE.cols != w_k || dEo.rows != dE.rows || dEo.cols != w_n || !Ybelow || !colpart ||
      ldcolpart < dEo.cols || !aligned16(Ybelow) || (strideYbelow & 3) || !colpartE || ldcolpartE < dE.cols)
    return TNET_ERR_ARG;
  GemmP p{};
  p.M = dE.rows; p.N = w_n; p.K = dE.cols;
  p.A = E; p.lda = dE.stride; p.B = W; p.ldb = dW.stride; p.C = Eo; p.ldc = dEo.stride;
  p.alpha = 1.f; p.beta = 0.f;
  p.aux = Ybelow; p.ldaux = strideYbelow;
  p.cpart = colpart; p.ldcpart = ldcolpart;
  int st = check_common(p);
  if (st) return st;
  if (p.M <= 0 || p.N <= 0 || forced_cfg() >= 0 || g_reserve > 0) return TNET_ERR_UNSUPPORTED;
  if ((long)cdiv(p.M, 64) * cdiv(p.N, 128) < 200) return TNET_ERR_UNSUPPORTED;
  if (4L * p.M * p.lda >= (1L << 32) || 4L * (bt ? (long)p.K : (long)p.N) * p.ldb >= (1L << 32))
    return TNET_ERR_UNSUPPORTED;
  const int slabs = cs_slabs(dE.rows);
  if (slabs != cdiv(dE.rows, CS_ROWS) || (dE.cols & 3) || (dE.stride & 3) || !aligned16(E)) return TNET_ERR_UNSUPPORTED;
  p.group = g_group > 0 ? g_group : 8;
  p.early_issue = g_early;
  p.wt = g_wt;
  const int na = cdiv(p.M, 64) * cdiv(p.N, 128), ncb = cdiv(dE.cols, CS_COLS * 4);
  const unsigned grid = (unsigned)(na + ncb * slabs);
  if (bt) {
// ... 545 lines not shown
```

### nnet-asr_amd/tnet_amd/__init__.py

```python
from __future__ import annotations

import ctypes as C
from typing import Callable, Optional, Sequence

import numpy as np

from . import formats
from ._lib import HOST_ALLREDUCE_FN, LIB_PATH, MatrixDim, TnetError, check, check_ptr, header_symbols, lib

__all__ = ["DeviceArray", "Network", "Objective", "Trainer", "RbmTrainer", "RnnTrainer", "Comm", "TnetError", "synchronize",
           "FeatureReader", "htk_read", "mask_match", "mlf_lookup",
           "pad_stride",
           "device_count", "version", "LIB_PATH", "header_symbols", "formats"]


def pad_stride(cols: int) -> int:
    return ((cols + 63) // 64) * 64 if cols else 0


def device_count() -> int:
    n = C.c_int(0)
    lib().tnet_device_count(C.byref(n))
    return n.value

# ... 80 lines not shown
        ni = np.array([a for a, _ in self.blocks], np.int32)
        no = np.array([b for _, b in self.blocks], np.int32)
        p = C.c_void_p()
        check(lib().tnet_discrete_plan_create(ni.ctypes.data, no.ctypes.data, len(self.blocks), C.byref(p)),
              "discrete_plan_create")
        self.ptr = p.value
        self.floats = int(lib().tnet_discrete_plan_floats(self.ptr))
        self.layout = []
        for k in range(len(self.blocks)):
            off, ld = C.c_long(), C.c_int()
            check(lib().tnet_discrete_plan_block(self.ptr, k, C.byref(off), C.byref(ld)), "discrete_plan_block")
            self.layout.append((off.value, ld.value))

    def pack(self, Ws, fill: float = 0.0) -> np.ndarray:
        out = np.full(self.floats, fill, np.float32)
        for W, (ni, no), (off, ld) in zip(Ws, self.blocks, self.layout):
            out[off:off + ni * ld].reshape(ni, ld)[:, :no] = np.asarray(W, np.float32).reshape(ni, no)
        return out

    def unpack(self, packed: np.ndarray):
        packed = np.asarray(packed).reshape(-1)
        return [packed[off:off + ni * ld].reshape(ni, ld)[:, :no].copy()
                for (ni, no), (off, ld) in zip(self.blocks, self.layout)]

    def padding(self, packed: np.ndarray) -> np.ndarray:
        packed = np.asarray(packed).reshape(-1)
        parts = [packed[off:off + ni * ld].reshape(ni, ld)[:, no:].reshape(-1)
                 for (ni, no), (off, ld) in zip(self.blocks, self.layout)]
        return np.concatenate(parts)

    def __del__(self):
        try:
            if getattr(self, "ptr", None):
                lib().tnet_synchronize()
                lib().tnet_discrete_plan_free(self.ptr)
                self.ptr = None
        except Exception:
            pass


class Network:

    def __init__(self, path: Optional[str] = None, text: Optional[str] = None):
        if path is not None:
            self.h = check_ptr(lib().tnet_net_read(path.encode()), "tnet_net_read")
        elif text is not None:
            self.h = check_ptr(lib().tnet_net_read_text(text.encode()), "tnet_net_read_text")
        else:
            raise ValueError("path or text required")

    @classmethod
    def from_layers(cls, layers, precision: int = 9) -> "Network":
        import io
        buf = io.StringIO()
        formats.write_nnet(layers, buf, precision=precision)
        return cls(text=buf.getvalue())

    def write(self, path: str) -> None:
        check(lib().tnet_net_write(self.h, path.encode()), "tnet_net_write")

    def components(self):
        out = []
        for i in range(lib().tnet_net_num_components(self.h)):
            tag = C.create_string_buffer(64)
            ni, no = C.c_int(), C.c_int()
            check(lib().tnet_net_component(self.h, i, tag, 64, C.byref(ni), C.byref(no)), "component")
            out.append((tag.value.decode(), ni.value, no.value))
        return out

    @property
    def n_in(self) -> int:
        return self.components()[0][1]

    @property
    def n_out(self) -> int:
        return self.components()[-1][2]

    def get_params(self, i: int):
        tag, ni, no = self.components()[i]
        W = np.empty((ni, no), np.float32)
        b = np.empty(no, np.float32)
        check(lib().tnet_net_get_params(self.h, i, W.ctypes.data, b.ctypes.data), "get_params")
        return W, b

    def linear_params(self):
        return [self.get_params(i) for i, c in enumerate(self.components()) if c[0] == "<biasedlinearity>"]

    def set_params(self, i: int, W: np.ndarray, b: np.ndarray) -> None:
        W = np.ascontiguousarray(W, np.float32)
        b = np.ascontiguousarray(b, np.float32)
        check(lib().tnet_net_set_params(self.h, i, W.ctypes.data, b.ctypes.data), "set_params")

    def set_learn_rate(self, lr: float, factors: Optional[str] = None) -> None:
        check(lib().tnet_net_set_learn_rate(self.h, lr, factors.encode() if factors else None), "learn_rate")

    def set_momentum(self, m: float) -> None:
        check(lib().tnet_net_set_momentum(self.h, m), "momentum")

    def set_weightcost(self, wc: float) -> None:
        check(lib().tnet_net_set_weightcost(self.h, wc), "weightcost")

    def set_grad_div_frm(self, div: bool) -> None:
        check(lib().tnet_net_set_grad_div_frm(self.h, int(div)), "graddivfrm")

    def propagate(self, X: DeviceArray, Y: Optional[DeviceArray] = None) -> DeviceArray:
        if Y is None:
            Y = DeviceArray(X.rows, self.n_out)
        check(lib().tnet_net_propagate(self.h, X.ptr, X.rows, X.stride, Y.ptr, Y.stride), "propagate")
        return Y

    def backpropagate(self, E: DeviceArray) -> None:
        check(lib().tnet_net_backpropagate(self.h, E.ptr, E.rows, E.stride), "backpropagate")

    def train_bunch(self, obj: "Objective", X: DeviceArray, labels: DeviceArray, train: bool = True) -> None:
        check(lib().tnet_net_train_bunch(self.h, obj.h, X.ptr, X.rows, X.stride, labels.ptr, int(train)),
              "train_bunch")

    def recurrent_params(self, i: int = 0):
        _, ni, no = self.components()[i]
        W = np.empty((ni + no, no), np.float32)
        b = np.empty(no, np.float32)
        check(lib().tnet_net_recurrent_get(self.h, i, W.ctypes.data, b.ctypes.data), "recurrent_get")
        return W, b

    def shared_params(self, i: int = 0):
        _, ni, no = self.components()[i]
        n = C.c_int()
        check(lib().tnet_net_shared_get(self.h, i, None, None, C.byref(n)), "shared_get")
        W = np.empty((ni // n.value, no // n.value), np.float32)
        b = np.empty(no // n.value, np.float32)
        check(lib().tnet_net_shared_get(self.h, i, W.ctypes.data, b.ctypes.data, None), "shared_get")
        return W, b, n.value

    def set_shared_params(self, i: int, W=None, b=None) -> None:
        W = None if W is None else np.ascontiguousarray(W, np.float32)
        b = None if b is None else np.ascontiguousarray(b, np.float32)
        if W is not None or b is not None:
            Wc, bc, _ = self.shared_params(i)
            if (W is not None and W.shape != Wc.shape) or (b is not None and b.shape != bc.shape):
                raise ValueError("set_shared_params: shape mismatch")
        check(lib().tnet_net_shared_set(self.h, i, None if W is None else W.ctypes.data,
                                        None if b is None else b.ctypes.data), "shared_set")

    def discrete_blocks(self, i: int = 0):
        n = C.c_int()
        check(lib().tnet_net_discrete_blocks(self.h, i, C.byref(n), None, None), "discrete_blocks")
        ni, no = np.zeros(n.value, np.int32), np.zeros(n.value, np.int32)
        check(lib().tnet_net_discrete_blocks(self.h, i, None, ni.ctypes.data, no.ctypes.data), "discrete_blocks")
        return [(int(a), int(b)) for a, b in zip(ni, no)]

    def discrete_params(self, i: int = 0):
        Ws = []
        for k, (ni, no) in enumerate(self.discrete_blocks(i)):
            W = np.empty((ni, no), np.float32)
            check(lib().tnet_net_discrete_get(self.h, i, k, W.ctypes.data, None), "discrete_get")
            Ws.append(W)
        b = np.empty(self.components()[i][2], np.float32)
        check(lib().tnet_net_discrete_get(self.h, i, 0, None, b.ctypes.data), "discrete_get")
        return Ws, b

    def set_discrete_params(self, i: int, Ws=None, b=None) -> None:
        blocks = self.discrete_blocks(i)
        if Ws is not None:
            if len(Ws) != len(blocks):
                raise ValueError("set_discrete_params: block count mismatch")
            for k, (W, shape) in enumerate(zip(Ws, blocks)):
# ... 435 lines not shown
```

### nnet-asr_amd/tnet_amd/_lib.py

```python
from __future__ import annotations

import ctypes as C
import os
import re

_HERE = os.path.dirname(os.path.abspath(__file__))
LIB_PATH = os.path.join(os.path.dirname(_HERE), "lib", "libtnet_amd.so")
if os.environ.get("TNET_DIAG_STAMP_LIB"):
    _v = os.environ["TNET_DIAG_STAMP_LIB"]
    LIB_PATH = os.path.join(os.path.dirname(_HERE), "lib", "libtnet_amd_stamp" + ("" if _v == "1" else "_" + _v) + ".so")
if os.environ.get("TNET_LIB_VARIANT"):
    LIB_PATH = os.path.join(os.path.dirname(_HERE), "lib", "libtnet_amd_" + os.environ["TNET_LIB_VARIANT"] + ".so")
INCLUDE_DIR = os.path.join(os.path.dirname(os.path.dirname(_HERE)), "include")

_lib = None


class TnetError(RuntimeError):
    pass


class MatrixDim(C.Structure):
    _fields_ = [("rows", C.c_int), ("cols", C.c_int), ("stride", C.c_int)]


vp = C.c_void_p
i32 = C.c_int
f32 = C.c_float
i64 = C.c_long
dp = C.POINTER(C.c_double)

_SIGS = {
    "tnet_status_str": (C.c_char_p, [i32]),
    "tnet_version": (C.c_char_p, []),
    "tnetF_set_const": (i32, [vp, f32, MatrixDim, vp]),
    "tnetF_apply_log": (i32, [vp, MatrixDim, vp]),
    "tnetF_apply_mask": (i32, [vp, vp, MatrixDim, MatrixDim, vp]),
    "tnetF_apply_l1": (i32, [vp, f32, MatrixDim, vp]),
    "tnetF_scale_cols": (i32, [vp, vp, MatrixDim, vp]),
    "tnetF_scale_rows": (i32, [vp, vp, MatrixDim, vp]),
    "tnetF_add_scaled": (i32, [f32, vp, i32, f32, vp, MatrixDim, vp]),
    "tnetF_add_scaled_row": (i32, [f32, vp, f32, vp, MatrixDim, vp]),
    "tnetF_mul_elem": (i32, [vp, vp, i32, MatrixDim, vp]),
    "tnetF_log_elem": (i32, [vp, MatrixDim, vp]),
    "tnet_col_sum_workspace": (i64, [MatrixDim]),
    "tnetF_add_col_sum": (i32, [f32, vp, f32, vp, MatrixDim, vp, vp]),
    "tnetF_sigmoid": (i32, [vp, vp, MatrixDim, vp]),
    "tnetF_diff_sigmoid": (i32, [vp, vp, vp, MatrixDim, vp]),
    "tnetF_softmax": (i32, [vp, vp, MatrixDim, vp]),
    "tnetF_check_class": (i32, [vp, vp, vp, MatrixDim, vp]),
    "tnetF_expand": (i32, [vp, vp, vp, MatrixDim, MatrixDim, vp]),
    "tnetF_rearrange": (i32, [vp, vp, vp, MatrixDim, MatrixDim, vp]),
    "tnetF_randomize": (i32, [vp, vp, vp, MatrixDim, MatrixDim, vp]),
    "tnet_block_linearity": (i32, [vp, MatrixDim, vp, MatrixDim, vp, MatrixDim, vp]),
    "tnet_gather_i32": (i32, [vp, vp, vp, i32, vp]),
    "tnet_gather_bunch": (i32, [vp, vp, vp, vp, vp, MatrixDim, MatrixDim, vp]),
    "tnet_sgemm": (i32, [C.c_char, C.c_char, i32, i32, i32, f32, vp, i32, vp, i32, f32, vp, i32, vp]),
    "tnet_gemm_config": (i32, [C.c_char_p]),
    "tnet_gemm_reserve": (i32, [i32]),
    "tnet_affine_fwd": (i32, [vp, MatrixDim, vp, MatrixDim, vp, vp, MatrixDim, i32, vp]),
    "tnet_affine_fwd_sample": (i32, [vp, MatrixDim, vp, MatrixDim, vp, vp, MatrixDim, vp, i32, vp, vp, vp, vp, vp]),
    "tnet_affine_bwd": (i32, [vp, MatrixDim, vp, MatrixDim, vp, i32, vp, MatrixDim, i32, vp]),
    "tnet_affine_update": (i32, [vp, MatrixDim, vp, MatrixDim, vp, MatrixDim, vp, i32, f32, f32, f32, vp]),
    "tnet_colsum_slabs": (i32, [i32]),
    "tnet_affine_update_row": (i32, [vp, i32, vp, i32, vp, i32, vp, i32, vp, vp, f32, f32, f32, vp]),
    "tnet_affine_bwd_update_row": (i32, [vp, i32, vp, i32, vp, i32, vp, i32, vp, vp, f32, f32, f32, vp, vp, vp, vp]),
    "tnet_gemv_rowvec_cat": (i32, [vp, i32, vp, i32, vp, vp, i32, vp, vp, i32, i32, vp, vp]),
    "tnet_gemv_rowvec_softmax_xent": (i32, [vp, i32, vp, i32, vp, vp, vp, vp, i32, vp, vp, vp, vp]),
    "tnet_colsum_slab_sums": (i32, [vp, MatrixDim, vp, i32, vp]),
    "tnet_affine_softmax_xent": (i32, [vp, MatrixDim, vp, MatrixDim, vp, vp, vp, i32, vp, i32, vp, i32, vp, vp, i32,
                                       vp]),
    "tnet_affine_grad_bias": (i32, [vp, MatrixDim, vp, MatrixDim, vp, MatrixDim, vp, i32, vp, vp]),
    "tnet_affine_grad_bwd_pair": (i32, [vp, MatrixDim, vp, MatrixDim, vp, MatrixDim, vp, i32, vp, vp, MatrixDim, vp,
                                        MatrixDim, vp, i32, vp, MatrixDim, vp, i32, vp]),
    "tnet_affine_grad_bias_gather": (i32, [vp, MatrixDim, vp, MatrixDim, vp, MatrixDim, vp, i32, vp, vp, MatrixDim, vp,
                                           MatrixDim, vp, MatrixDim, vp, i32, vp, vp, vp, vp, vp, vp, MatrixDim,
                                           MatrixDim, vp]),
    "tnet_sgd_update_multi": (i32, [vp, i32, f32, f32, vp]),
    "tnet_affine_bwd_colsum": (i32, [vp, MatrixDim, vp, MatrixDim, vp, i32, vp, MatrixDim, vp, i32, vp]),
    "tnet_affine_bwd_colsum_slabs": (i32, [vp, MatrixDim, vp, MatrixDim, vp, i32, vp, MatrixDim, vp, i32, vp, i32,
                                           vp]),
    "tnet_affine_bwd_colsum_t": (i32, [vp, MatrixDim, vp, MatrixDim, vp, i32, vp, MatrixDim, vp, i32, vp]),
    "tnet_affine_bwd_colsum_slabs_t": (i32, [vp, MatrixDim, vp, MatrixDim, vp, i32, vp, MatrixDim, vp, i32, vp, i32,
                                             vp]),
    "tnet_affine_update_bwd_pair_t": (i32, [vp, MatrixDim, vp, MatrixDim, vp, MatrixDim, vp, i32, f32, f32, f32, vp,
                                            i32, vp, vp, vp, MatrixDim, vp, MatrixDim, vp, i32, vp, MatrixDim, vp, i32,
                                            vp]),
    "tnet_weight_shadow": (i32, [vp, MatrixDim, vp, i32]),
    "tnet_weight_shadow_kept": (i32, [vp]),
    "tnet_transpose": (i32, [vp, MatrixDim, vp, i32, vp]),
    "tnet_affine_update_bias": (i32, [vp, MatrixDim, vp, MatrixDim, vp, MatrixDim, vp, i32, f32, f32, f32, vp, i32,
                                      vp, vp, vp]),
    "tnet_affine_update_bias_pair": (i32, [vp, MatrixDim, vp, MatrixDim, vp, MatrixDim, vp, i32, f32, f32, f32, vp, i32,
                                           vp, vp, vp, MatrixDim, vp, MatrixDim, vp, MatrixDim, vp, i32, f32, f32,
                                           f32, vp, i32, vp, vp, vp]),
    "tnet_affine_update_bias_gather": (i32, [vp, MatrixDim, vp, MatrixDim, vp, MatrixDim, vp, i32, f32, f32, f32, vp,
                                             i32, vp, vp, vp, MatrixDim, vp, MatrixDim, vp, MatrixDim, vp, i32, f32,
                                             f32, f32, vp, i32, vp, vp, vp, vp, vp, vp, vp, MatrixDim, MatrixDim, vp]),
    "tnet_affine_update_bwd_pair": (i32, [vp, MatrixDim, vp, MatrixDim, vp, MatrixDim, vp, i32, f32, f32, f32, vp, i32,
                                          vp, vp, vp, MatrixDim, vp, MatrixDim, vp, i32, vp, MatrixDim, vp, i32, vp]),
    "tnet_affine_grad": (i32, [vp, MatrixDim, vp, MatrixDim, vp, MatrixDim, vp]),
    "tnet_shared_fwd": (i32, [vp, MatrixDim, vp, MatrixDim, vp, i32, vp, MatrixDim, vp]),
    "tnet_shared_bwd": (i32, [vp, MatrixDim, vp, MatrixDim, i32, vp, MatrixDim, vp]),
    "tnet_shared_update": (i32, [vp, MatrixDim, vp, MatrixDim, i32, vp, MatrixDim, vp, i32, vp, vp, f32, f32, f32,
                                 vp]),
    "tnet_shared_grad": (i32, [vp, MatrixDim, vp, MatrixDim, i32, vp, MatrixDim, vp, vp]),
    "tnet_discrete_plan_create": (i32, [vp, vp, i32, C.POINTER(vp)]),
    "tnet_discrete_plan_free": (i32, [vp]),
    "tnet_discrete_plan_floats": (i64, [vp]),
    "tnet_discrete_plan_blocks": (i32, [vp]),
    "tnet_discrete_plan_block": (i32, [vp, i32, C.POINTER(i64), C.POINTER(i32)]),
    "tnet_discrete_loop_routing": (i32, [i32]),
    "tnet_discrete_fwd": (i32, [vp, MatrixDim, vp, vp, vp, vp, MatrixDim, vp]),
    "tnet_discrete_bwd": (i32, [vp, MatrixDim, vp, vp, vp, MatrixDim, vp]),
    "tnet_discrete_update": (i32, [vp, MatrixDim, vp, MatrixDim, vp, vp, vp, vp, vp, f32, f32, f32, vp]),
    "tnet_discrete_grad": (i32, [vp, MatrixDim, vp, MatrixDim, vp, vp, vp, vp]),
    "tnet_sparse_grad": (i32, [vp, MatrixDim, vp, MatrixDim, vp, MatrixDim, vp, vp]),
    "tnet_sparse_apply": (i32, [vp, MatrixDim, vp, i32, vp, i32, vp, i32, vp, i32, i64, i64, f32, f32, f32, f32, vp]),
    "tnet_sparse_mask_pack": (i32, [vp, MatrixDim, vp, i32, vp]),
    "tnet_sparse_mask_unpack": (i32, [vp, i32, vp, MatrixDim, vp]),
    "tnet_sparse_update": (i32, [vp, MatrixDim, vp, MatrixDim, vp, MatrixDim, vp, i32, vp, i32, vp, i32, vp, vp, f32,
                                 f32, f32, f32, vp]),
    "tnet_sparse_update_form": (i32, [i32]),
    "tnet_sparse_mask_update": (i32, [vp, MatrixDim, vp, i32, vp, i32, f32, f32, f32, vp]),
    "tnet_sgd_update": (i32, [vp, vp, vp, i64, f32, f32, f32, vp]),
    "tnet_bias_update": (i32, [vp, MatrixDim, vp, vp, vp, f32, f32, vp, vp]),
    "tnet_softmax_xent": (i32, [vp, MatrixDim, vp, vp, i32, vp, i32, vp, vp]),
    "tnet_softmax_xent_dense": (i32, [vp, MatrixDim, vp, i32, vp, i32, vp, i32, vp, vp]),
    "tnet_mse": (i32, [vp, MatrixDim, vp, i32, vp, i32, vp, vp]),
    "tnet_stats_fetch": (i32, [vp, dp, dp, vp]),
    "tnet_last_error": (C.c_char_p, []),
    "tnet_device_count": (i32, [C.POINTER(i32)]),
    "tnet_select_gpu": (i32, [i32]),
    "tnet_synchronize": (i32, []),
    "tnet_stream": (vp, []),
    "tnet_malloc": (i32, [C.POINTER(vp), C.c_size_t]),
    "tnet_free": (i32, [vp]),
    "tnet_memcpy_h2d": (i32, [vp, vp, C.c_size_t]),
    "tnet_memcpy_d2h": (i32, [vp, vp, C.c_size_t]),
    "tnet_memcpy_d2d": (i32, [vp, vp, C.c_size_t]),
    "tnet_memset": (i32, [vp, i32, C.c_size_t]),
    "tnet_set_profile": (i32, [i32]),
    "tnet_profile_report": (i32, [C.c_char_p, i32]),
    "tnet_kernel_timing": (i32, [i32]),
    "tnet_kernel_timing_filter": (i32, [C.c_char_p]),
    "tnet_kernel_timing_report": (i32, [C.c_char_p, i32]),
    "tnet_timer_start": (i32, []),
    "tnet_timer_stop": (i32, [C.POINTER(f32)]),
    "tnet_net_read": (vp, [C.c_char_p]),
    "tnet_net_read_text": (vp, [C.c_char_p]),
    "tnet_net_write": (i32, [vp, C.c_char_p]),
    "tnet_net_free": (i32, [vp]),
    "tnet_net_num_components": (i32, [vp]),
    "tnet_net_component": (i32, [vp, i32, C.c_char_p, i32, C.POINTER(i32), C.POINTER(i32)]),
    "tnet_net_get_params": (i32, [vp, i32, vp, vp]),
    "tnet_net_set_params": (i32, [vp, i32, vp, vp]),
    "tnet_net_set_learn_rate": (i32, [vp, f32, C.c_char_p]),
    "tnet_net_set_momentum": (i32, [vp, f32]),
    "tnet_net_set_weightcost": (i32, [vp, f32]),
    "tnet_net_set_grad_div_frm": (i32, [vp, i32]),
    "tnet_net_propagate": (i32, [vp, vp, i32, i32, vp, i32]),
    "tnet_net_backpropagate": (i32, [vp, vp, i32, i32]),
    "tnet_net_train_bunch": (i32, [vp, vp, vp, i32, i32, vp, i32]),
    "tnet_net_keep_output": (i32, [vp, i32]),
    "tnet_net_output": (i32, [vp, i32, vp, i32]),
    "tnet_obj_create": (vp, [i32]),
    "tnet_obj_free": (i32, [vp]),
    "tnet_obj_evaluate": (i32, [vp, vp, i32, i32, i32, vp, i32, vp, i32]),
    "tnet_obj_evaluate_labels": (i32, [vp, vp, i32, i32, i32, vp, vp, i32]),
    "tnet_obj_stats": (i32, [vp, dp, C.POINTER(i64), dp]),
    "tnet_obj_report": (i32, [vp, C.c_char_p, i32]),
    "tnet_obj_reset": (i32, [vp]),
    "tnet_trainer_create": (vp, [vp, vp, i32, i32, i64, i32, i32]),
    "tnet_trainer_free": (i32, [vp]),
    "tnet_trainer_add_utterance": (i32, [vp, vp, i32, i32, i32, vp]),
    "tnet_trainer_finish": (i32, [vp]),
    "tnet_trainer_steps": (i64, [vp]),
    "tnet_trainer_replay": (i32, [vp, i64]),
    "tnet_trainer_prefill": (i64, [vp, vp, i32, i32, i32, vp]),
    "tnet_debug_fail_train_bunch": (i32, [i64]),
    "tnet_trainer_set_comm": (i32, [vp, vp]),
    "tnet_trainer_trace": (i32, [vp, i32]),
    "tnet_trainer_set_transform": (i32, [vp, vp, i32, i32]),
    "tnet_reader_create": (vp, [C.c_char_p, i32, i32, i32, i32, i32, vp, C.c_char_p, C.c_char_p, C.c_char_p,
                                C.c_char_p, i32, i32]),
    "tnet_reader_create_norm": (vp, [C.c_char_p, i32, i32, i32, i32, i32, vp, C.c_char_p, C.c_char_p, C.c_char_p,
                                     C.c_char_p, C.c_char_p, C.c_char_p, C.c_char_p, C.c_char_p, C.c_char_p, i32,
                                     i32]),
    "tnet_reader_free": (i32, [vp]),
    "tnet_reader_size": (i64, [vp]),
    "tnet_reader_next": (i32, [vp, C.POINTER(vp), C.POINTER(i32), C.POINTER(i32), C.POINTER(vp), C.POINTER(i32),
                              C.POINTER(i32), C.POINTER(i32), C.c_char_p, i32]),
    "tnet_reader_rewind": (i32, [vp]),
    "tnet_htk_read": (i32, [C.c_char_p, i32, i32, i32, vp, i64, C.POINTER(i32), C.POINTER(i32), C.POINTER(i32),
                           C.POINTER(i32)]),
    "tnet_mask_match": (i32, [C.c_char_p, C.c_char_p, C.c_char_p, i32]),
    "tnet_mlf_lookup": (i32, [vp, i32, vp, i32, vp]),
    "tnet_trainer_add_reader": (i64, [vp, vp, i64]),
    "tnet_comm_unique_id": (i32, [C.c_char_p]),
    "tnet_comm_create": (vp, [i32, i32, C.c_char_p]),
    "tnet_comm_free": (i32, [vp]),
    "tnet_comm_allreduce_host": (i32, [vp, dp, i32]),
    "tnet_comm_allreduce_device": (i32, [vp, vp, i64]),
    "tnet_comm_capture": (i32, [vp, i32]),
    "tnet_comm_captured": (i64, [vp]),
    "tnet_comm_captured_block": (i32, [vp, i64, vp, vp, i64, C.POINTER(i64)]),
    "tnet_comm_transport_ranks": (i32, [vp, C.POINTER(i32)]),
    "tnet_comm_create_host": (vp, [i32, i32, vp, vp]),
    "tnet_net_rbm_get": (i32, [vp, i32, vp, vp, vp, vp]),
    "tnet_net_rbm_set": (i32, [vp, i32, vp, vp, vp, i32, i32]),
    "tnet_net_rbm_update": (i32, [vp, i32, vp, vp, vp, vp, i32, i32, i32]),
    "tnet_rbm_trainer_create": (vp, [vp, i32, i32, i64, i32, f32, f32, f32]),
    "tnet_rbm_trainer_free": (i32, [vp]),
    "tnet_rbm_trainer_add_utterance": (i32, [vp, vp, i32, i32, i32]),
    "tnet_rbm_trainer_finish": (i32, [vp]),
    "tnet_rbm_trainer_steps": (i64, [vp]),
    "tnet_rbm_trainer_stats": (i32, [vp, dp, C.POINTER(i64)]),
    "tnet_rbm_trainer_report": (i32, [vp, C.c_char_p, i32]),
    "tnet_rbm_trainer_prefill": (i64, [vp, vp, i32, i32, i32]),
    "tnet_rbm_trainer_replay": (i32, [vp, i64]),
    "tnet_net_recurrent_get": (i32, [vp, i32, vp, vp]),
    "tnet_net_recurrent_set": (i32, [vp, i32, vp, vp]),
    "tnet_net_shared_get": (i32, [vp, i32, vp, vp, vp]),
    "tnet_net_shared_set": (i32, [vp, i32, vp, vp]),
    "tnet_net_discrete_blocks": (i32, [vp, i32, vp, vp, vp]),
    "tnet_net_discrete_get": (i32, [vp, i32, i32, vp, vp]),
    "tnet_net_discrete_set": (i32, [vp, i32, i32, vp, vp]),
    "tnet_net_set_l1": (i32, [vp, f32]),
    "tnet_net_sparse_get": (i32, [vp, i32, vp, vp, vp, vp, C.POINTER(i64)]),
    "tnet_net_sparse_set": (i32, [vp, i32, vp, vp, vp]),
    "tnet_net_sparse_thresholds": (i32, [vp, i32, f32, f32]),
    "tnet_net_sparse_update_mask": (i32, [vp, i32]),
    "tnet_rnn_trainer_create": (vp, [vp, vp, i32, i32]),
    "tnet_rnn_trainer_free": (i32, [vp]),
    "tnet_rnn_trainer_utterance": (i32, [vp, vp, i32, i32, i32, vp]),
    "tnet_rnn_trainer_frames": (i64, [vp]),
    "tnet_gemv_workspace": (i64, [i32, i32]),
    "tnet_gemv_rowvec": (i32, [vp, i32, vp, i32, vp, vp, i32, i32, vp, vp]),
    "tnet_gemv_rows": (i32, [vp, i32, i32, i32, i32, vp, vp, f32, vp, vp]),
# ... 114 lines not shown
```

Measured before the change: 1.022 million frames/s.

## Fuse transposed weight shadow write into forward GEMM B-tile loads

```diff
diff --git a/include/tnet_kernels.h b/include/tnet_kernels.h
--- a/include/tnet_kernels.h
+++ b/include/tnet_kernels.h
@@ -116,6 +116,8 @@
 int tnet_weight_shadow(const float* W, TnetMatrixDim dW, float* Wt, int ldwt);
 int tnet_weight_shadow_kept(const float* W);
 int tnet_transpose(const float* A, TnetMatrixDim dA, float* T, int ldt, void* stream);
+int tnet_affine_fwd_shadow(const float* X, TnetMatrixDim dX, const float* W, TnetMatrixDim dW, const float* b,
+                           float* Y, TnetMatrixDim dY, int act, float* Wt, int ldwt, void* stream);
 int tnet_affine_update_bias_gather(const float* X, TnetMatrixDim dX, const float* E, TnetMatrixDim dE, float* W,
                                    TnetMatrixDim dW, float* corrW, int strideCorr, float scale, float mmt, float l2,
                                    const float* colpart, int ldcolpart, float* b, float* corr_b, const float* X2,
diff --git a/include/tnet_train.h b/include/tnet_train.h
--- a/include/tnet_train.h
+++ b/include/tnet_train.h
@@ -44,6 +44,7 @@
 int tnet_net_component(TnetNetwork* net, int i, char* tag, int cap, int* n_in, int* n_out);
 int tnet_net_get_params(TnetNetwork* net, int i, float* W, float* b);
 int tnet_net_set_params(TnetNetwork* net, int i, const float* W, const float* b);
+int tnet_net_get_shadow(TnetNetwork* net, int i, float* Wt, int* state);
 int tnet_net_set_learn_rate(TnetNetwork* net, float lr, const char* factors);
 int tnet_net_set_momentum(TnetNetwork* net, float mmt);
 int tnet_net_set_weightcost(TnetNetwork* net, float wc);
diff --git a/nnet-asr_amd/csrc/host/capi.cpp b/nnet-asr_amd/csrc/host/capi.cpp
--- a/nnet-asr_amd/csrc/host/capi.cpp
+++ b/nnet-asr_amd/csrc/host/capi.cpp
@@ -227,6 +227,13 @@
   if (b) L.Bias().CopyToHost(b);
   TRY_END
 }
+int tnet_net_get_shadow(TnetNetwork* h, int i, float* Wt, int* state) {
+  TRY_BEGIN const CuBiasedLinearity& L = linear(h, i);
+  const CuMatrix<BaseFloat>& T = L.ShadowRO();
+  if (state) *state = (L.HasShadow() ? 1 : 0) | (L.ShadowValid() ? 2 : 0) | (L.FwdShadow() ? 4 : 0);
+  if (Wt && L.HasShadow()) T.CopyToHost(Wt, T.Cols());
+  TRY_END
+}
 int tnet_net_set_params(TnetNetwork* h, int i, const float* W, const float* b) {
   TRY_BEGIN CuBiasedLinearity& L = linear(h, i);
   if (W) {
diff --git a/nnet-asr_amd/csrc/host/culayers.cpp b/nnet-asr_amd/csrc/host/culayers.cpp
--- a/nnet-asr_amd/csrc/host/culayers.cpp
+++ b/nnet-asr_amd/csrc/host/culayers.cpp
@@ -132,6 +132,35 @@
                                     (int)mLinearityT.Stride()));
   mShadowKey = mLinearity.pCUData();
   mShadowOn = true;
+  mFwdShadow = false;
+}
+
+void CuBiasedLinearity::UseFwdShadow() {
+  if (mFwdRefused) {
+    UseShadow();
+    return;
+  }
+  if (!mShadowOn || mLinearityT.Rows() != mLinearity.Cols() || mLinearityT.Cols() != mLinearity.Rows()) {
+    mLinearityT.Init(mLinearity.Cols(), mLinearity.Rows());
+    mShadowValid = false;
+  }
+  if (mShadowKey) (void)tnet_weight_shadow(mShadowKey, TnetMatrixDim{}, nullptr, 0);
+  mShadowKey = nullptr;
+  mShadowOn = true;
+  mFwdShadow = true;
+}
+
+bool CuBiasedLinearity::PropagateShadow(const CuMatrix<BaseFloat>& X, CuMatrix<BaseFloat>& Y, int act) {
+  const int st = tnet_affine_fwd_shadow(X.pCUData(), X.Dim(), mLinearity.pCUData(), mLinearity.Dim(), mBias.pCUData(),
+                                        Y.pCUData(), Y.Dim(), act, mLinearityT.pCUData(), (int)mLinearityT.Stride(), S);
+  if (st == TNET_ERR_UNSUPPORTED) {
+    mFwdRefused = true;
+    UseShadow();
+    return false;
+  }
+  TNET_SAFE_CALL(st);
+  mShadowValid = true;
+  return true;
 }
 
 void CuBiasedLinearity::DropShadowKey() {
diff --git a/nnet-asr_amd/csrc/host/culayers.h b/nnet-asr_amd/csrc/host/culayers.h
--- a/nnet-asr_amd/csrc/host/culayers.h
+++ b/nnet-asr_amd/csrc/host/culayers.h
@@ -43,6 +43,11 @@
   void UseShadow();
   const CuMatrix<BaseFloat>& ShadowForBwd();
   bool HasShadow() const { return mShadowOn; }
+  void UseFwdShadow();
+  bool FwdShadow() const { return mShadowOn && mFwdShadow; }
+  const CuMatrix<BaseFloat>& ShadowRO() const { return mLinearityT; }
+  bool ShadowValid() const { return mShadowOn && mShadowValid; }
+  bool PropagateShadow(const CuMatrix<BaseFloat>& X, CuMatrix<BaseFloat>& Y, int act);
   CuVector<BaseFloat>& Bias() { return mBias; }
   CuMatrix<BaseFloat>& LinearityCorrection() { return mLinearityCorrection; }
   CuVector<BaseFloat>& BiasCorrection() { return mBiasCorrection; }
@@ -72,6 +77,7 @@
   CuVector<BaseFloat> mGradB;
   CuMatrix<BaseFloat> mLinearityT;
   bool mShadowOn = false, mShadowValid = false;
+  bool mFwdShadow = false, mFwdRefused = false;
   const float* mShadowKey = nullptr;
   void DropShadowKey();
   void NoteUpdate() { mShadowValid = mShadowOn && tnet_weight_shadow_kept(mLinearity.pCUData()) == 1; }
diff --git a/nnet-asr_amd/csrc/host/cunetwork.cpp b/nnet-asr_amd/csrc/host/cunetwork.cpp
--- a/nnet-asr_amd/csrc/host/cunetwork.cpp
+++ b/nnet-asr_amd/csrc/host/cunetwork.cpp
@@ -306,6 +306,8 @@
 
 static const bool g_dp_pair = !(getenv("TNET_DP_PAIR") && getenv("TNET_DP_PAIR")[0] == '0');
 
+static const int kBwdShadowDefault = 1;
+
 void CuNetwork::TrainBunch(const CuMatrix<BaseFloat>& X, const CuVector<int>& labels, CuObjectiveFunction& obj,
                            bool train, GradExchange* exchange) {
   if (g_fail_train_bunch > 0 && --g_fail_train_bunch == 0) Error("CuNetwork::TrainBunch: injected fault");
@@ -336,11 +338,17 @@
     }
   }
   mNetComponents.front()->SetInput(X);
-  static const int use_shadow = getenv("TNET_BWD_SHADOW") ? atoi(getenv("TNET_BWD_SHADOW")) : 2;
+  static const int use_shadow = getenv("TNET_BWD_SHADOW") ? atoi(getenv("TNET_BWD_SHADOW")) : kBwdShadowDefault;
+  static const int fwd_shadow = getenv("TNET_FWD_SHADOW") ? atoi(getenv("TNET_FWD_SHADOW")) : 1;
+  static const bool fuse_top = !(getenv("TNET_FUSED_TOP") && getenv("TNET_FUSED_TOP")[0] == '0');
   const bool shadows = use_shadow > 0 && train && !exchange;
   if (shadows)
-    for (int l = 1; l < (use_shadow == 2 ? nl - 1 : nl); l++)
-      static_cast<CuBiasedLinearity*>(mNetComponents[2 * l])->UseShadow();
+    for (int l = 1; l < (use_shadow == 2 ? nl - 1 : nl); l++) {
+      auto* lin = static_cast<CuBiasedLinearity*>(mNetComponents[2 * l]);
+      const bool top = l == nl - 1, fused = top && fuse_top && lin->GetNOutputs() <= TNET_AFFINE_SOFTMAX_MAX_N;
+      if ((top ? fwd_shadow > 0 : fwd_shadow > 1) && !fused) lin->UseFwdShadow();
+      else lin->UseShadow();
+    }
 
   CuComponent* smx = mNetComponents.back();
   float* yout = nullptr;
@@ -366,7 +374,6 @@
     CuMatrix<BaseFloat>& dst = last ? lin->Output() : actc->Output();
     dst.Init(rows, lin->GetNOutputs());
     const std::string shape = std::to_string(lin->GetNInputs()) + "x" + std::to_string(lin->GetNOutputs());
-    static const bool fuse_top = !(getenv("TNET_FUSED_TOP") && getenv("TNET_FUSED_TOP")[0] == '0');
     if (last && fuse_top && lin->GetNOutputs() <= TNET_AFFINE_SOFTMAX_MAX_N) {
       float* cp = nullptr;
       int ldcp = 0;
@@ -389,8 +396,10 @@
       }
     }
     KTScope kt("gemm_fwd:" + shape, 2.0 * rows * lin->GetNInputs() * lin->GetNOutputs());
-    TNET_SAFE_CALL(tnet_affine_fwd(act->pCUData(), act->Dim(), lin->LinearityRO().pCUData(), lin->LinearityRO().Dim(),
-                                   lin->Bias().pCUData(), dst.pCUData(), dst.Dim(), last ? 0 : 1, S));
+    if (!(shadows && lin->FwdShadow() && lin->PropagateShadow(*act, dst, last ? 0 : 1)))
+      TNET_SAFE_CALL(tnet_affine_fwd(act->pCUData(), act->Dim(), lin->LinearityRO().pCUData(),
+                                     lin->LinearityRO().Dim(), lin->Bias().pCUData(), dst.pCUData(), dst.Dim(),
+                                     last ? 0 : 1, S));
     act = &dst;
     acts[l + 1] = &dst;
   }
diff --git a/nnet-asr_amd/csrc/kernels/gemm_f32.hip b/nnet-asr_amd/csrc/kernels/gemm_f32.hip
--- a/nnet-asr_amd/csrc/kernels/gemm_f32.hip
+++ b/nnet-asr_amd/csrc/kernels/gemm_f32.hip
@@ -53,6 +53,7 @@
   unsigned* rz[4];
   float* skws;
   float* Ct; long ldct;
+  float* Wt; long ldwt;
 };
 
 
@@ -563,7 +564,8 @@
 constexpr int gemm16_smem_floats() {
   return S * (BM + BN) * BK;
 }
-template <int BM, int BN, int BK, int WM, int WN, int S, int SP, bool A_KC, bool B_KC, int EPI_T, bool PX>
+template <int BM, int BN, int BK, int WM, int WN, int S, int SP, bool A_KC, bool B_KC, int EPI_T, bool PX,
+          bool TS = false>
 __device__ __forceinline__ void gemm16_body(const GemmP& p_in, float* __restrict__ smem, const int bid_x) {
   constexpr bool SKM = EPI_T >= kEpiStreamK;
   constexpr int EPI = SKM ? EPI_T - kEpiStreamK : EPI_T;
@@ -1059,19 +1061,61 @@
         return v;
       };
       constexpr int WV = (DD - 2) * NR;
-      auto wait_slot = [&](f32x4 (&q)[NR]) {
+      auto wait_slot_x = [&](f32x4 (&q)[NR], auto xs) {
+        constexpr int WX = WV + decltype(xs)::value;
+        static_assert(WX < 64, "vmcnt range");
         if constexpr (NR == 6)
           asm volatile("s_waitcnt vmcnt(%6)" : "+v"(q[0]), "+v"(q[1]), "+v"(q[2]), "+v"(q[3]), "+v"(q[4]), "+v"(q[5])
-                       : "n"(WV));
+                       : "n"(WX));
         else if constexpr (NR == 8)
           asm volatile("s_waitcnt vmcnt(%8)"
                        : "+v"(q[0]), "+v"(q[1]), "+v"(q[2]), "+v"(q[3]), "+v"(q[4]), "+v"(q[5]), "+v"(q[6]), "+v"(q[7])
-                       : "n"(WV));
+                       : "n"(WX));
         else
           asm volatile("s_waitcnt vmcnt(%12)"
                        : "+v"(q[0]), "+v"(q[1]), "+v"(q[2]), "+v"(q[3]), "+v"(q[4]), "+v"(q[5]), "+v"(q[6]), "+v"(q[7]),
                          "+v"(q[8]), "+v"(q[9]), "+v"(q[10]), "+v"(q[11])
-                       : "n"(WV));
+                       : "n"(WX));
+      };
+      auto wait_slot = [&](f32x4 (&q)[NR]) { wait_slot_x(q, std::integral_constant<int, 0>{}); };
+      constexpr int TSN = 4;
+      static_assert(!TS || (!B_KC && VN == 4 && NRB == 4 && !CKC && !SKM),
+                    "shadow writer: one 4x4 block of an n-contiguous B per lane");
+      int ts_lo = 0, ts_hi = 0;
+      unsigned ts_off[TSN] = {0u, 0u, 0u, 0u};
+      __amdgpu_buffer_rsrc_t ts_rs = rB;
+      if constexpr (TS) {
+        const int nsh = WM * nbm, me = (bm / BM) * WM + wid / WN;
+        if (bn + wn0 < N) {
+          ts_lo = (int)((long)me * nch / nsh);
+          ts_hi = (int)((long)(me + 1) * nch / nsh);
+        }
+        const int ncol = max(min(bn + wn0 + VN * li, N - VN), 0);
+#pragma unroll
+        for (int e = 0; e < TSN; ++e) ts_off[e] = 4u * (unsigned)((ncol + e) * (int)p.ldwt + 4 * lg);
+        ts_rs = __builtin_amdgcn_make_buffer_rsrc((void*)p.Wt, (short)0, (int)(4 * ((long)(N - 1) * p.ldwt + K)),
+                                                  0x00020000);
+      }
+      auto ts_store = [&](f32x4 (&q)[NR], int c) {
+#pragma unroll
+        for (int e = 0; e < TSN; ++e) {
+          const f32x4 v = {q[NRA][e], q[NRA + 1][e], q[NRA + 2][e], q[NRA + 3][e]};
+#ifdef TNET_GEMM_DIAG_SHADOWWT
+          __builtin_amdgcn_raw_buffer_store_b128(__builtin_bit_cast(u32x4, v), ts_rs, (int)ts_off[e], c * 64, 16);
+#else
+          __builtin_amdgcn_raw_buffer_store_b128(__builtin_bit_cast(u32x4, v), ts_rs, (int)ts_off[e], c * 64, 0);
+#endif
+        }
+      };
+      auto wait_ts = [&](f32x4 (&q)[NR], int c) {
+        const int ns = max(min(c, ts_hi) - max(c - (DD - 2), ts_lo), 0);
+        if (ns == 0) wait_slot_x(q, std::integral_constant<int, 0>{});
+        else if (ns == 1) wait_slot_x(q, std::integral_constant<int, TSN>{});
+        else if (DD <= 4 || ns == 2) wait_slot_x(q, std::integral_constant<int, 2 * TSN>{});
+        else if (ns == 3) wait_slot_x(q, std::integral_constant<int, (DD > 4 ? 3 : 0) * TSN>{});
+        else if (ns == 4) wait_slot_x(q, std::integral_constant<int, (DD > 4 ? 4 : 0) * TSN>{});
+        else if (ns == 5) wait_slot_x(q, std::integral_constant<int, (DD > 4 ? 5 : 0) * TSN>{});
+        else wait_slot_x(q, std::integral_constant<int, (DD > 4 ? 6 : 0) * TSN>{});
       };
       const int pperm = 4 * (4 * li + lg);
       auto perm = [&](f32x4& v) {
@@ -1092,13 +1136,19 @@
 #pragma unroll
         for (int t = 0; t < NKC; ++t) perm(ring[0][kc_reg(t)]);
       }
-      for (int c0 = 0; c0 < nch; c0 += DD) {
+      auto turn = [&](const int c0, auto tsg) __attribute__((always_inline)) {
+        constexpr bool TSG = decltype(tsg)::value;
 #pragma unroll
         for (int j = 0; j < DD; ++j) {
           const int cn = min(c0 + j + DD - 1, nch - 1);
           if constexpr (!CKC) {
             __builtin_amdgcn_sched_barrier(0);
-            wait_slot(ring[j]);
+            if constexpr (TSG) {
+              wait_ts(ring[j], c0 + j);
+              if (c0 + j >= ts_lo && c0 + j < ts_hi) ts_store(ring[j], c0 + j);
+            } else {
+              wait_slot(ring[j]);
+            }
             __builtin_amdgcn_sched_barrier(0);
           }
           int mi = 0;
@@ -1129,6 +1179,14 @@
                 }
                 ++mi;
               }
+        }
+      };
+      for (int c0 = 0; c0 < nch; c0 += DD) {
+        if constexpr (TS) {
+          if (c0 + DD > ts_lo && c0 < ts_hi + DD - 2) turn(c0, std::true_type{});
+          else turn(c0, std::false_type{});
+        } else {
+          turn(c0, std::false_type{});
         }
       }
       asm volatile("s_waitcnt vmcnt(0)" ::: "memory");
@@ -1355,6 +1413,15 @@
     }
   }
 
+  if constexpr (TS) {
+    static_assert(DIR && SP >= 5 && SP <= 6, "the shadow writer lives in the a<D> direct forms");
+    const int k0 = nfull * BK, Kt = K - k0, ncols = min(BN, N - bn);
+    if (bm == 0 && Kt > 0)
+      for (int u = threadIdx.x; u < Kt * ncols; u += NT) {
+        const int k = k0 + u / ncols, n = bn + u % ncols;
+        p.Wt[(long)n * p.ldwt + k] = p.B[(long)k * p.ldb + n];
+      }
+  }
   if constexpr (SKM) {
     if (p.ksplit > 1) {
       constexpr int SLICE = BM * BN;
@@ -1682,12 +1749,13 @@
   gemm16_body<BM, BN, 64, 2, 2, 2, 0, A_KC, B_KC, kEpiStreamK + EPI, PX>(q, smem, v >> 1);
 }
 
-template <int BM, int BN, int BK, int WM, int WN, int S, int SP, bool A_KC, bool B_KC, int EPI_T, bool PX = false>
+template <int BM, int BN, int BK, int WM, int WN, int S, int SP, bool A_KC, bool B_KC, int EPI_T, bool PX = false,
+          bool TS = false>
 __global__ __launch_bounds__((WM * WN + (SP == 2)) * 64)
 __attribute__((amdgpu_waves_per_eu((WM * WN + (SP == 2) + 3) / 4, (WM * WN + (SP == 2) + 3) / 4)))
 void gemm16_kernel(const GemmP p_in) {
   __shared__ __attribute__((aligned(16))) float smem[gemm16_smem_floats<BM, BN, BK, S, EPI_T, PX>()];
-  gemm16_body<BM, BN, BK, WM, WN, S, SP, A_KC, B_KC, EPI_T, PX>(p_in, smem, blockIdx.x);
+  gemm16_body<BM, BN, BK, WM, WN, S, SP, A_KC, B_KC, EPI_T, PX, TS>(p_in, smem, blockIdx.x);
 }
 
 template <int BMA, int BNA, bool AKA, bool BKA, int EPIA, bool PXA, int BMB, int BNB, bool AKB, bool BKB, int EPIB,
@@ -2341,6 +2409,59 @@
   return GemmPlan{cfg, ks};
 }
 
+static int direct_cfg(int cfg, const GemmP& p) {
+  if (g_direct > 0 && forced_cfg() < 0) {
+    if (cfg == CFG_m64x128k64s2) return (g_direct == 3 || p.K <= 512) ? CFG_m64x128a4 : CFG_m64x128a8;
+    if (cfg == CFG_m128x128k64s2) return CFG_m128x128a4;
+    if (cfg == CFG_m128x256k32s3 && g_direct == 4) return CFG_m128x256a2;
+  }
+  return cfg;
+}
+
+template <int BM, int BN, int IL, int EPI>
+static int launch_fwd_shadow_cfg(const GemmP& p, hipStream_t st) {
+  constexpr int BK = 64;
+  const long extA = (long)p.M * p.lda, extB = (long)BK * p.ldb + p.N;
+  if (4 * extA >= (1L << 32) || 4 * extB >= (1L << 32)) return TNET_ERR_UNSUPPORTED;
+  const int nfull = p.K / BK;
+  auto a16p = [](const void* v) { return ((uintptr_t)v & 15) == 0; };
+  if (nfull < 1 || p.N % 4 || (IL == 6 && nfull % 2) || (p.lda & 3) || (p.ldb & 3) || !a16p(p.A) || !a16p(p.B) ||
+      4 * (long)p.M * p.lda >= (1L << 31) || 4 * (long)p.K * p.ldb >= (1L << 31) ||
+      4 * (long)p.N * p.ldwt >= (1L << 31))
+    return TNET_ERR_UNSUPPORTED;
+  const unsigned tiles = (unsigned)((long)cdiv(p.M, BM) * cdiv(p.N, BN));
+  GemmP q = p;
+  q.early_issue = g_early;
+  q.wt = g_wt;
+  constexpr bool PXK = BM == 64 && BN == 128 && EPI == EPI_BIAS_SIG;
+  if constexpr (PXK) {
+    if (px_exact<BM, BN, EPI>(p)) {
+      gemm16_kernel<BM, BN, BK, 2, 2, 2, IL, true, false, EPI, true, true><<<tiles, 256, 0, st>>>(q);
+      return TNET_OK;
+    }
+  }
+  gemm16_kernel<BM, BN, BK, 2, 2, 2, IL, true, false, EPI, false, true><<<tiles, 256, 0, st>>>(q);
+  return TNET_OK;
+}
+template <int EPI>
+static int launch_fwd_shadow(const GemmP& p_in, hipStream_t st) {
+  static const int noload = getenv("TNET_GEMM_DIAG") ? atoi(getenv("TNET_GEMM_DIAG")) : 0;
+  GemmP p = p_in;
+  p.diag_noload = noload;
+  p.group = g_group > 0 ? g_group : 8;
+  const GemmPlan pl = plan_gemm<true>(p, epi_splittable(EPI));
+  if (pl.ks > 1 || g_reserve > 0) return TNET_ERR_UNSUPPORTED;
+  int st_ = TNET_ERR_UNSUPPORTED;
+  switch (direct_cfg(pl.cfg, p)) {
+    case CFG_m64x128a4: st_ = launch_fwd_shadow_cfg<64, 128, 5, EPI>(p, st); break;
+    case CFG_m64x128a8: st_ = launch_fwd_shadow_cfg<64, 128, 6, EPI>(p, st); break;
+    case CFG_m128x128a4: st_ = launch_fwd_shadow_cfg<128, 128, 5, EPI>(p, st); break;
+    default: break;
+  }
+  if (st_ == TNET_OK) TNET_LAUNCH_CHECK();
+  return st_;
+}
+
 template <bool A_KC, bool B_KC, int EPI>
 static int launch_gemm(const GemmP& p_in, hipStream_t st) {
   if constexpr (EPI == EPI_DSIG_CS) {
@@ -2367,12 +2488,7 @@
     return TNET_OK;
   }
   int rcfg = cfg;
-  if (g_direct > 0 && forced_cfg() < 0 && !B_KC) {
-    if (cfg == CFG_m64x128k64s2)
-      rcfg = (g_direct == 3 || p.K <= 512) ? CFG_m64x128a4 : CFG_m64x128a8;
-    else if (cfg == CFG_m128x128k64s2) rcfg = CFG_m128x128a4;
-    else if (cfg == CFG_m128x256k32s3 && g_direct == 4) rcfg = CFG_m128x256a2;
-  }
+  if (!B_KC) rcfg = direct_cfg(cfg, p);
   if (g_kc >= 2 && forced_cfg() < 0 && A_KC && B_KC && cfg == CFG_m64x128k64s2) rcfg = CFG_m64x128c8;
   if constexpr (!A_KC && !B_KC && (EPI == EPI_SGD_B || EPI == EPI_SGD))
     if (forced_cfg() < 0 && cfg == CFG_m64x64k32s4w41 && upd64_direct(p)) rcfg = CFG_m64x64a4;
@@ -2755,6 +2871,29 @@
       p, na, V, dV, H, dH, B, nvb, vb, cvb, hb, chb, scale, mmt, mse_stats, nhb, g, ng);
   TNET_LAUNCH_CHECK();
   return TNET_OK;
+}
+
+extern "C" int tnet_affine_fwd_shadow(const float* X, TnetMatrixDim dX, const float* W, TnetMatrixDim dW,
+                                      const float* b, float* Y, TnetMatrixDim dY, int act, float* Wt, int ldwt,
+                                      void* stream) {
+  if (dX.cols != dW.rows || dY.rows != dX.rows || dY.cols != dW.cols || !b || !Wt || act < 0 || act > 3)
+    return TNET_ERR_ARG;
+  GemmP p{};
+  p.M = dX.rows; p.N = dW.cols; p.K = dX.cols;
+  p.A = X; p.lda = dX.stride; p.B = W; p.ldb = dW.stride; p.C = Y; p.ldc = dY.stride;
+  p.bias = b;
+  p.Wt = Wt; p.ldwt = ldwt;
+  int st = check_common(p);
+  if (st) return st;
+  if (p.M <= 0 || p.N <= 0 || p.K <= 0 || act > 1) return TNET_ERR_UNSUPPORTED;
+  if (!aligned16(Wt) || (ldwt & 3) || ldwt < p.K) return TNET_ERR_UNSUPPORTED;
+  if (any_overlap({span_of(Wt, p.N, ldwt, sizeof(float))},
+                  {span_of(X, p.M, p.lda, sizeof(float)), span_of(W, p.K, p.ldb, sizeof(float)),
+                   span_of(Y, p.M, p.ldc, sizeof(float)), span_of(b, 1, p.N, sizeof(float))}))
+    return TNET_ERR_UNSUPPORTED;
+  if (act == 0 && top_split_ok(p)) return TNET_ERR_UNSUPPORTED;
+  if (act == 1) return launch_fwd_shadow<EPI_BIAS_SIG>(p, (hipStream_t)stream);
+  return launch_fwd_shadow<EPI_BIAS>(p, (hipStream_t)stream);
 }
 
 extern "C" int tnet_affine_bwd(const float* E, TnetMatrixDim dE, const float* W, TnetMatrixDim dW,
diff --git a/nnet-asr_amd/tnet_amd/__init__.py b/nnet-asr_amd/tnet_amd/__init__.py
--- a/nnet-asr_amd/tnet_amd/__init__.py
+++ b/nnet-asr_amd/tnet_amd/__init__.py
@@ -186,6 +186,13 @@
         b = np.empty(no, np.float32)
         check(lib().tnet_net_get_params(self.h, i, W.ctypes.data, b.ctypes.data), "get_params")
         return W, b
+
+    def get_shadow(self, i: int):
+        _, ni, no = self.components()[i]
+        Wt = np.empty((no, ni), np.float32)
+        state = C.c_int(0)
+        check(lib().tnet_net_get_shadow(self.h, i, Wt.ctypes.data, C.byref(state)), "get_shadow")
+        return (Wt if state.value & 1 else None), state.value
 
     def linear_params(self):
         return [self.get_params(i) for i, c in enumerate(self.components()) if c[0] == "<biasedlinearity>"]
diff --git a/nnet-asr_amd/tnet_amd/_lib.py b/nnet-asr_amd/tnet_amd/_lib.py
--- a/nnet-asr_amd/tnet_amd/_lib.py
+++ b/nnet-asr_amd/tnet_amd/_lib.py
@@ -89,6 +89,7 @@
     "tnet_weight_shadow": (i32, [vp, MatrixDim, vp, i32]),
     "tnet_weight_shadow_kept": (i32, [vp]),
     "tnet_transpose": (i32, [vp, MatrixDim, vp, i32, vp]),
+    "tnet_affine_fwd_shadow": (i32, [vp, MatrixDim, vp, MatrixDim, vp, vp, MatrixDim, i32, vp, i32, vp]),
     "tnet_affine_update_bias": (i32, [vp, MatrixDim, vp, MatrixDim, vp, MatrixDim, vp, i32, f32, f32, f32, vp, i32,
                                       vp, vp, vp]),
     "tnet_affine_update_bias_pair": (i32, [vp, MatrixDim, vp, MatrixDim, vp, MatrixDim, vp, i32, f32, f32, f32, vp, i32,
@@ -155,6 +156,7 @@
     "tnet_net_component": (i32, [vp, i32, C.c_char_p, i32, C.POINTER(i32), C.POINTER(i32)]),
     "tnet_net_get_params": (i32, [vp, i32, vp, vp]),
     "tnet_net_set_params": (i32, [vp, i32, vp, vp]),
+    "tnet_net_get_shadow": (i32, [vp, i32, vp, C.POINTER(i32)]),
     "tnet_net_set_learn_rate": (i32, [vp, f32, C.c_char_p]),
     "tnet_net_set_momentum": (i32, [vp, f32]),
     "tnet_net_set_weightcost": (i32, [vp, f32]),
```

Measured after the change: 1.004 million frames/s. 0.982x the previous value.
